# tensorflow/lingvo

Hardware: AMD Instinct MI355X
Metric: train step examples/sec (whole node), Librispeech Conformer-L (higher is better)
Workload: dtype bf16; 1 GPU; model=Conformer-L (17 blocks, d=512, h=8, kernel 32) + LSTM attention decoder, global_batch=512, seq_len=1200, parallelism=dp1, step_mode=hipgraph

## Files before the change

### lingvo_amd/core/py_utils.py

```python

from __future__ import annotations

import contextlib
import math
import threading
from typing import Any, List, Optional, Sequence, Tuple, Union

import torch

from lingvo_amd.core.hyperparams import Params
from lingvo_amd.core.nested_map import NestedMap


class WeightInit:

  @staticmethod
  def _Spec(method: str, scale: float) -> Params:
    p = Params()
    p.Define('method', method, 'Initialization method.')
    p.Define('scale', scale, 'Initialization scale.')
    return p

  @staticmethod
  def Gaussian(scale: float = 1.0) -> Params:
    return WeightInit._Spec('gaussian', scale)

  @staticmethod
  def Uniform(scale: float = 1.0) -> Params:
    return WeightInit._Spec('uniform', scale)

  @staticmethod
  def Constant(scale: float = 0.0) -> Params:
    return WeightInit._Spec('constant', scale)

  @staticmethod
  def Xavier(scale: float = 1.0) -> Params:
    return WeightInit._Spec('xavier', scale)

  @staticmethod
  def GeoMeanXavier(scale: float = 1.0) -> Params:
    return WeightInit._Spec('geo_mean_xavier', scale)

  @staticmethod
  def TruncatedGaussian(scale: float = 1.0) -> Params:
    return WeightInit._Spec('truncated_gaussian', scale)

  @staticmethod
  def GaussianSqrtDim(scale: float = 1.0) -> Params:
    return WeightInit._Spec('gaussian_sqrt_dim', scale)

  @staticmethod
  def UniformSqrtDim(scale: float = 1.0) -> Params:
    return WeightInit._Spec('uniform_sqrt_dim', scale)

  @staticmethod
  def UniformUnitScaling(scale: float = 1.0) -> Params:
    return WeightInit._Spec('uniform_unit_scaling', scale)

  @staticmethod
  def TruncatedGaussianSqrtFanIn(scale: float = 1.0) -> Params:
    return WeightInit._Spec('truncated_gaussian_sqrt_fanin', scale)

  @staticmethod
  def TruncatedGaussianSqrtFanOut(scale: float = 1.0) -> Params:
    return WeightInit._Spec('truncated_gaussian_sqrt_fanout', scale)


def WeightParams(shape: Sequence[int],
                 init: Optional[Params] = None,
                 dtype: torch.dtype = torch.float32,
                 collections: Optional[List[str]] = None) -> Params:
  p = Params()
  p.Define('shape', list(shape), 'Weight shape.')
  p.Define('init', init or WeightInit.Xavier(1.0), 'Initialization spec.')
  p.Define('dtype', dtype, 'Weight dtype.')
  p.Define('collections', collections or [], 'Weight collections.')
  return p


def _FanInFanOut(shape: Sequence[int]) -> Tuple[int, int]:
  if not shape:
    return 1, 1
  if len(shape) == 1:
    return shape[0], shape[0]
  receptive = 1
  for d in shape[:-2]:
    receptive *= d
  return shape[-2] * receptive, shape[-1] * receptive


def InitWeight(shape: Sequence[int], spec: Params,
               generator: Optional[torch.Generator] = None,
               dtype: torch.dtype = torch.float32) -> torch.Tensor:
  method, scale = spec.method, spec.scale
  shape = list(shape)
  dim0 = shape[0] if shape else 1
  fan_in, fan_out = _FanInFanOut(shape)

  def randn():
    return torch.randn(shape, generator=generator, dtype=torch.float32)

  def rand():
    return torch.rand(shape, generator=generator, dtype=torch.float32) * 2 - 1

  if method == 'constant':
    w = torch.full(shape, float(scale), dtype=torch.float32)
  elif method == 'gaussian':
    w = randn() * scale
  elif method == 'uniform':
    w = rand() * scale
  elif method == 'gaussian_sqrt_dim':
    w = randn() * (scale / math.sqrt(max(dim0, 1)))
  elif method == 'uniform_sqrt_dim':
    w = rand() * (scale / math.sqrt(max(dim0, 1)))
  elif method == 'xavier':
    limit = scale * math.sqrt(6.0 / (fan_in + fan_out))
    w = rand() * limit
  elif method == 'geo_mean_xavier':
    limit = scale * math.sqrt(3.0 / math.sqrt(fan_in * fan_out))
    w = rand() * limit
  elif method == 'uniform_unit_scaling':
    w = rand() * (scale * math.sqrt(3.0 / max(fan_in, 1)))
  elif method in ('truncated_gaussian', 'truncated_gaussian_sqrt_fanin',
                  'truncated_gaussian_sqrt_fanout'):
    std = scale
    if method.endswith('fanin'):
      std = scale / math.sqrt(max(fan_in, 1))
    elif method.endswith('fanout'):
      std = scale / math.sqrt(max(fan_out, 1))
    w = torch.empty(shape, dtype=torch.float32)
    torch.nn.init.trunc_normal_(w, std=std, a=-2 * std, b=2 * std,
                                generator=generator)
  else:
    raise ValueError(f'Unknown init method {method!r}')
  return w.to(dtype)


_RNG_STATE = threading.local()


def _GetRngStack() -> List[NestedMap]:
  if not hasattr(_RNG_STATE, 'stack'):
    _RNG_STATE.stack = [NestedMap(global_seed=1234, step=0, op_counter=[0])]
  return _RNG_STATE.stack


@contextlib.contextmanager
def StepSeedScope(global_seed: int, step: int):
  stack = _GetRngStack()
  stack.append(NestedMap(global_seed=int(global_seed), step=int(step),
                         op_counter=[0]))
  if torch.cuda.is_available():
    from lingvo_amd.ops import dropout as dropout_ops
    dropout_ops.SetStepSeed(int(step), int(global_seed))
  try:
    yield
  finally:
    stack.pop()


def GenerateStepSeedPair(op_seed: Optional[int] = None) -> Tuple[int, int]:
  top = _GetRngStack()[-1]
  if op_seed is None:
    op_seed = top.op_counter[0]
    top.op_counter[0] += 1
  mixed = (top.global_seed * 1000003 + op_seed) & 0x7FFFFFFF
  return mixed, top.step


def MakeStepGenerator(device: Union[str, torch.device],
                      op_seed: Optional[int] = None) -> torch.Generator:
  s1, s2 = GenerateStepSeedPair(op_seed)
  g = torch.Generator(device=device)
  g.manual_seed((s1 * 2654435761 + s2) & 0x7FFFFFFFFFFFFFFF)
  return g


def DeterministicDropout(x: torch.Tensor, keep_prob: float,
                         op_seed: Optional[int] = None,
                         act: str = 'NONE') -> torch.Tensor:
  if keep_prob >= 1.0:
    if act == 'SWISH':
      return torch.nn.functional.silu(x)
    if act == 'RELU':
      return torch.relu(x)
    return x
  if x.is_cuda and x.numel() % 8 == 0:
    from lingvo_amd.ops import dropout as dropout_ops
    s1, _ = GenerateStepSeedPair(op_seed)
    return dropout_ops.dropout(x, keep_prob, s1, act=act)
  if act == 'SWISH':
    x = torch.nn.functional.silu(x)
  elif act == 'RELU':
    x = torch.relu(x)
  g = MakeStepGenerator(x.device, op_seed)
  mask = (torch.rand(x.shape, generator=g, device=x.device,
                     dtype=torch.float32) < keep_prob)
  return x * mask.to(x.dtype) / keep_prob


def DeterministicDropoutAdd(x: torch.Tensor, keep_prob: float,
                            residual: torch.Tensor,
                            op_seed: Optional[int] = None,
                            scale: float = 1.0,
                            paddings: Optional[torch.Tensor] = None
                            ) -> torch.Tensor:
  if keep_prob >= 1.0:
    if scale != 1.0:
      x = x * scale
    if paddings is not None:
      x = ApplyPadding(paddings, x)
    return residual + x
  if x.is_cuda and x.numel() % 8 == 0 and \
      (paddings is None or x.shape[-1] % 8 == 0):
    from lingvo_amd.ops import dropout as dropout_ops
    s1, _ = GenerateStepSeedPair(op_seed)
    return dropout_ops.dropout(x, keep_prob, s1, residual=residual,
                               scale=scale, paddings=paddings)
  if scale != 1.0:
    x = x * scale
  if paddings is not None:
    x = ApplyPadding(paddings, x)
  return residual + DeterministicDropout(x, keep_prob, op_seed)


def PaddingsFromLengths(lengths: torch.Tensor, maxlen: int) -> torch.Tensor:
  pos = torch.arange(maxlen, device=lengths.device)[None, :]
  return (pos >= lengths[:, None]).float()


def LengthsFromPaddings(paddings: torch.Tensor) -> torch.Tensor:
  return (1.0 - paddings).sum(dim=1).round().long()


def ApplyPadding(padding: torch.Tensor, x: torch.Tensor,
                 padded_value: float = 0.0) -> torch.Tensor:
  while padding.dim() < x.dim():
    padding = padding.unsqueeze(-1)
  padding = padding.to(x.dtype)
  if padded_value == 0.0:
    return x * (1.0 - padding)
  return x * (1.0 - padding) + padded_value * padding


def PadSequenceDimension(x: torch.Tensor, length: int, pad_val: float = 0.0,
                         axis: int = 1) -> torch.Tensor:
  cur = x.shape[axis]
  if cur == length:
    return x
  if cur > length:
    raise ValueError(f'Cannot pad dim {axis} from {cur} down to {length}')
  pad_shape = list(x.shape)
  pad_shape[axis] = length - cur
  pad = torch.full(pad_shape, pad_val, dtype=x.dtype, device=x.device)
  return torch.cat([x, pad], dim=axis)


def ConcatenatePaddedSequences(x: torch.Tensor, y: torch.Tensor,
                               px: torch.Tensor, py: torch.Tensor
                               ) -> Tuple[torch.Tensor, torch.Tensor]:
  b = x.shape[0]
  lx = LengthsFromPaddings(px)
  ly = LengthsFromPaddings(py)
  tot = int((lx + ly).max().item())
  feat = x.shape[2:]
  out = torch.zeros((b, tot) + tuple(feat), dtype=x.dtype, device=x.device)
  pout = torch.ones((b, tot), dtype=px.dtype, device=px.device)
  for i in range(b):
    n1, n2 = int(lx[i]), int(ly[i])
    out[i, :n1] = x[i, :n1]
    out[i, n1:n1 + n2] = y[i, :n2]
    pout[i, :n1 + n2] = 0.0
  return out, pout


def TrimTrailingPaddings(x: torch.Tensor, paddings: torch.Tensor):
  lengths = LengthsFromPaddings(paddings)
  max_len = int(lengths.max().item()) if lengths.numel() else 0
  max_len = max(max_len, 1)
  return x[:, :max_len], paddings[:, :max_len]


def ReversePaddedSequence(x: torch.Tensor,
                          paddings: torch.Tensor) -> torch.Tensor:
  b, t = paddings.shape
  lengths = LengthsFromPaddings(paddings).to(torch.long)
  pos = torch.arange(t, device=x.device).unsqueeze(0).expand(b, t)
  rev = (lengths.unsqueeze(1) - 1 - pos).clamp_min(0)
  idx = torch.where(pos < lengths.unsqueeze(1), rev, pos)
  shaped = idx.reshape(b, t, *([1] * (x.dim() - 2))).expand_as(x)
  return torch.gather(x, 1, shaped)


def ShiftLeft(x: torch.Tensor, shift: int,
              pad_val: float = 0.0) -> torch.Tensor:
  if shift <= 0:
    return x
  pad = x.new_full((x.shape[0], shift, *x.shape[2:]), pad_val)
  return torch.cat([x[:, shift:], pad], dim=1)


def MixByWeight(fns, weights, seed: Optional[int] = None):
  import random as _random
  rng = _random.Random(seed)
  total = float(sum(weights))
  r = rng.uniform(0.0, total)
  acc = 0.0
  for i, (fn, w) in enumerate(zip(fns, weights)):
    acc += float(w)
    if r <= acc:
      return fn(), i
  return fns[-1](), len(fns) - 1


def SplitRecursively(x, num_splits: int, axis: int = -1):
  if isinstance(x, torch.Tensor):
    assert x.shape[axis] % num_splits == 0
    return list(x.chunk(num_splits, dim=axis))
  if isinstance(x, (list, tuple)):
    split_elems = [SplitRecursively(e, num_splits, axis) for e in x]
    return [type(x)(parts[i] for parts in split_elems)
            for i in range(num_splits)]
  if isinstance(x, NestedMap):
    flat = x.Flatten()
    split_flat = [SplitRecursively(e, num_splits, axis) for e in flat]
    return [x.Pack([parts[i] for parts in split_flat])
            for i in range(num_splits)]
  raise TypeError('Unsupported type for SplitRecursively: %r' % type(x))


def CheckNumerics(x: torch.Tensor, message: str = '') -> torch.Tensor:
  if not torch.isfinite(x).all():
    raise FloatingPointError(f'Tensor has NaN/Inf: {message}')
  return x


def HasNanOrInf(nmap_or_tensor) -> bool:
  if isinstance(nmap_or_tensor, torch.Tensor):
    return not bool(torch.isfinite(nmap_or_tensor).all())
  tensors = [v for v in nmap_or_tensor.Flatten()
             if isinstance(v, torch.Tensor) and v.is_floating_point()]
  return any(not bool(torch.isfinite(t).all()) for t in tensors)


def GlobalGradNorm(grads: List[torch.Tensor]) -> torch.Tensor:
  if not grads:
    return torch.zeros(())
  norms = torch._foreach_norm([g.detach() for g in grads], 2)
  return torch.stack([n.float() for n in norms]).norm(2)


def WeightedAvg(values: torch.Tensor, weights: torch.Tensor
                ) -> Tuple[torch.Tensor, torch.Tensor]:
  w = weights.float()
  total = w.sum()
  avg = (values.float() * w).sum() / total.clamp_min(1e-8)
  return avg, total


def WeightedAvgOfMetrics(metrics_list: List[NestedMap]) -> NestedMap:
  ret = NestedMap()
  if not metrics_list:
    return ret
  for name in metrics_list[0].keys():
    vals = torch.stack([torch.as_tensor(m[name][0]).float()
                        for m in metrics_list])
    wts = torch.stack([torch.as_tensor(m[name][1]).float()
                       for m in metrics_list])
    total_w = wts.sum()
    avg = (vals * wts).sum() / total_w.clamp_min(1e-8)
    ret[name] = (avg, total_w)
  return ret


def ToScalar(x) -> float:
  if isinstance(x, torch.Tensor):
    return float(x.detach().cpu().item())
  return float(x)


def AddVn(theta: NestedMap, vn_std: float) -> NestedMap:

  def add_noise(t):
    if isinstance(t, torch.Tensor) and t.is_floating_point() and \
        t.requires_grad:
      u = GraphSafeUniform(t.shape, t.device).clamp(1e-6, 1 - 1e-6)
      normal = torch.erfinv(2 * u - 1) * math.sqrt(2.0)
      return t + vn_std * normal.to(t.dtype)
    return t

  return theta.Transform(add_noise)


def GraphSafeUniform(shape, device, op_seed: Optional[int] = None
                     ) -> torch.Tensor:
  import math as _math
  n = 1
  for d in shape:
    n *= int(d)
  s1, s2 = GenerateStepSeedPair(op_seed)
  if not (isinstance(device, torch.device) and device.type == 'cuda') and \
      str(device) != 'cuda' and not str(device).startswith('cuda'):
    g = torch.Generator()
    g.manual_seed((s1 * 2654435761 + s2) & 0x7FFFFFFFFFFFFFFF)
    return torch.rand(shape, generator=g)
  from lingvo_amd.ops import dropout as dropout_ops
  buf = dropout_ops._StepSeedBuf(torch.device(device))

  def lshr(x, k):
    return (x >> k) & ((1 << (64 - k)) - 1)

  idx = torch.arange(n, device=device, dtype=torch.int64)
  h = (idx * 0x9E3779B97F4A7C15) ^ (buf + s1)
  h = h ^ lshr(h, 33)
  h = h * -0xAE502812AA7333
  h = h ^ lshr(h, 33)
  h = h * -0x3B314601E57A13AD
  h = h ^ lshr(h, 33)
  u = (h & 0x7FFFFFFF).float() / float(1 << 31)
  return u.reshape(shape)


def MatmulBias(x: torch.Tensor, w: torch.Tensor,
               b: Optional[torch.Tensor] = None) -> torch.Tensor:
  shape = x.shape
  x2 = x.reshape(-1, shape[-1])
  if b is None:
    out = torch.matmul(x2, w)
  else:
    out = torch.addmm(b, x2, w)
  return out.reshape(*shape[:-1], w.shape[-1])


def GlueFusion() -> bool:
  from lingvo_amd.ops import fusion
  return fusion.enabled()


def SetGlueFusion(enabled: bool) -> bool:
  from lingvo_amd.ops import fusion
  return fusion.set_enabled(enabled)


def _CanFuseLinearDropout(x, w, b, keep_prob) -> bool:
  return (GlueFusion() and b is not None and keep_prob < 1.0 and
          x.is_cuda and x.dtype == torch.bfloat16 and
          w.dtype == torch.bfloat16 and b.dtype == torch.bfloat16 and
          w.shape[-1] % 8 == 0 and x.numel() > 0)


def MatmulBiasDropout(x: torch.Tensor, w: torch.Tensor,
                      b: Optional[torch.Tensor], keep_prob: float,
                      op_seed: Optional[int] = None,
                      act: str = 'NONE') -> torch.Tensor:
  if _CanFuseLinearDropout(x, w, b, keep_prob):
    from lingvo_amd.ops import dropout as dropout_ops
    s1, _ = GenerateStepSeedPair(op_seed)
    return dropout_ops.linear_dropout(x, w, b, keep_prob, s1, act=act)
  return DeterministicDropout(MatmulBias(x, w, b), keep_prob, op_seed,
                              act=act)


def MatmulBiasDropoutAdd(x: torch.Tensor, w: torch.Tensor,
                         b: Optional[torch.Tensor], keep_prob: float,
                         residual: torch.Tensor,
                         op_seed: Optional[int] = None, scale: float = 1.0,
                         paddings: Optional[torch.Tensor] = None
                         ) -> torch.Tensor:
  if _CanFuseLinearDropout(x, w, b, keep_prob) and \
      residual.dtype == torch.bfloat16:
    from lingvo_amd.ops import dropout as dropout_ops
    s1, _ = GenerateStepSeedPair(op_seed)
    return dropout_ops.linear_dropout(x, w, b, keep_prob, s1,
                                      residual=residual, scale=scale,
                                      paddings=paddings)
  return DeterministicDropoutAdd(MatmulBias(x, w, b), keep_prob, residual,
                                 op_seed, scale=scale, paddings=paddings)


class Timer:

  def __init__(self):
    self._total = 0.0
    self._start = None

  def Start(self):
    import time
    self._start = time.perf_counter()
    return self

  def Stop(self):
    import time
    if self._start is not None:
      self._total += time.perf_counter() - self._start
      self._start = None
    return self

  def Duration(self) -> float:
    return self._total

  def __enter__(self):
    return self.Start()

  def __exit__(self, *a):
    self.Stop()


def SinkhornAssignment(scores: torch.Tensor, tau: float = 0.1,
                       n_iters: int = 20) -> torch.Tensor:
  log_alpha = scores / tau
  for _ in range(n_iters):
    log_alpha = log_alpha - torch.logsumexp(log_alpha, dim=-1,
                                            keepdim=True)
    log_alpha = log_alpha - torch.logsumexp(log_alpha, dim=-2,
                                            keepdim=True)
  return torch.exp(log_alpha)


def AssertShapeMatch(tensor: torch.Tensor, pattern) -> torch.Tensor:
  shape = tuple(tensor.shape)
  assert len(shape) == len(pattern), (shape, pattern)
  for got, want in zip(shape, pattern):
    assert want == -1 or got == want, (shape, pattern)
  return tensor


def AssertIdShape(*tensors: torch.Tensor) -> None:
  shapes = {tuple(t.shape) for t in tensors}
  assert len(shapes) == 1, shapes


def EstimateFlops(fn, *args) -> int:
  from torch.profiler import profile, ProfilerActivity
  with profile(activities=[ProfilerActivity.CPU],
               with_flops=True) as prof:
    fn(*args)
  return int(sum(e.flops for e in prof.key_averages() if e.flops))


def RandomPermutationSequence(num: int, batch: int,
                              op_seed: Optional[int] = None
                              ) -> torch.Tensor:
  keys = GraphSafeUniform((batch, num), 'cpu', op_seed)
  return keys.argsort(dim=1)


class CachedCall:

  def __init__(self, fn):
    self._fn = fn
    self._has = False
    self._val = None

  def __call__(self):
    if not self._has:
      self._val = self._fn()
      self._has = True
    return self._val
```

### lingvo_amd/layers/conformer.py

```python

from __future__ import annotations

import os
from typing import Optional

import torch
import torch.nn.functional as F

from lingvo_amd.core import py_utils
from lingvo_amd.core.base_layer import BaseLayer
from lingvo_amd.core.nested_map import NestedMap
from lingvo_amd.layers import attention as attention_lib
from lingvo_amd.layers import bn_layers
from lingvo_amd.layers import layers as lingvo_layers
from lingvo_amd.layers import transformer as transformer_lib
from lingvo_amd.ops import conv1d as conv1d_ops


class LConvLayer(BaseLayer):

  @classmethod
  def Params(cls):
    p = super().Params()
    p.Define('input_dim', 0, 'Model dim.')
    p.Define('kernel_size', 32, 'Depthwise conv kernel size.')
    p.Define('is_causal', False, 'Causal depthwise conv.')
    p.Define('conv_norm', 'group', "One of 'batch'|'group'|'layer'.")
    p.Define('num_groups', 32, 'Groups for group norm.')
    p.Define('dropout_prob', 0.0, 'Output dropout.')
    return p

  def __init__(self, params):
    super().__init__(params)
    p = self.p
    d = p.input_dim
    self.CreateChild('ln', lingvo_layers.LayerNorm.Params().Set(
        input_dim=d))
    self.CreateVariable('pw1_w', py_utils.WeightParams(
        [d, 2 * d], p.params_init, p.dtype))
    self.CreateVariable('pw1_b', py_utils.WeightParams(
        [2 * d], py_utils.WeightInit.Constant(0.0), p.dtype))
    self.CreateVariable('dw_w', py_utils.WeightParams(
        [p.kernel_size, d], p.params_init, p.dtype))
    self.CreateVariable('dw_b', py_utils.WeightParams(
        [d], py_utils.WeightInit.Constant(0.0), p.dtype))
    if p.conv_norm == 'batch':
      self.CreateChild('norm', bn_layers.BatchNormLayer.Params().Set(dim=d))
    elif p.conv_norm == 'group':
      self.CreateChild('norm', bn_layers.GroupNormLayer.Params().Set(
          dim=d, num_groups=p.num_groups))
    else:
      self.CreateChild('norm', lingvo_layers.LayerNorm.Params().Set(
          input_dim=d))
    self.CreateVariable('pw2_w', py_utils.WeightParams(
        [d, d], p.params_init, p.dtype))
    self.CreateVariable('pw2_b', py_utils.WeightParams(
        [d], py_utils.WeightInit.Constant(0.0), p.dtype))

  def FProp(self, theta: NestedMap, inputs: torch.Tensor,
            paddings: Optional[torch.Tensor] = None) -> torch.Tensor:
    p = self.p
    x, residual = transformer_lib.PreLn(self.ln, theta.ln, inputs)
    x = py_utils.MatmulBias(x, theta.pw1_w, theta.pw1_b)
    x = F.glu(x, dim=-1)
    if paddings is not None:
      x = py_utils.ApplyPadding(paddings, x)
    x = conv1d_ops.depthwise_conv1d(x, theta.dw_w, theta.dw_b,
                                    causal=p.is_causal)
    if p.conv_norm == 'layer':
      x = self.norm.FProp(theta.norm, x)
      if paddings is not None:
        x = py_utils.ApplyPadding(paddings, x)
      x = F.silu(x)
    elif p.conv_norm == 'group':
      x = self.norm.FProp(theta.norm, x, paddings, act='SILU')
    else:
      x = self.norm.FProp(theta.norm, x, paddings)
      x = F.silu(x)
    if p.dropout_prob and not self.do_eval:
      return py_utils.MatmulBiasDropoutAdd(
          x, theta.pw2_w, theta.pw2_b, 1.0 - p.dropout_prob, residual,
          paddings=paddings)
    x = py_utils.MatmulBias(x, theta.pw2_w, theta.pw2_b)
    if paddings is not None:
      x = py_utils.ApplyPadding(paddings, x)
    return residual + x

  def InitStreamState(self, batch: int, device, dtype) -> NestedMap:
    p = self.p
    return NestedMap(conv=torch.zeros(batch, p.kernel_size - 1,
                                      p.input_dim, device=device,
                                      dtype=dtype))

  def StreamStep(self, theta: NestedMap, inputs: torch.Tensor,
                 paddings: torch.Tensor, state: NestedMap):
    p = self.p
    assert p.is_causal, 'StreamStep requires a causal LConv'
    x = self.ln.FProp(theta.ln, inputs)
    x = py_utils.MatmulBias(x, theta.pw1_w, theta.pw1_b)
    x = F.glu(x, dim=-1)
    x = py_utils.ApplyPadding(paddings, x)
    full = torch.cat([state.conv.to(x.dtype), x], dim=1)
    y = conv1d_ops.depthwise_conv1d(full, theta.dw_w, theta.dw_b,
                                    causal=True)
    x = y[:, state.conv.shape[1]:]
    new_state = NestedMap(conv=full[:, -(p.kernel_size - 1):]
                          if p.kernel_size > 1 else state.conv)
    if p.conv_norm == 'layer':
      x = self.norm.FProp(theta.norm, x)
      x = py_utils.ApplyPadding(paddings, x)
    else:
      x = self.norm.FProp(theta.norm, x, paddings)
    x = F.silu(x)
    x = py_utils.MatmulBias(x, theta.pw2_w, theta.pw2_b)
    x = py_utils.ApplyPadding(paddings, x)
    return inputs + x, new_state


class ConformerLayer(BaseLayer):

  @classmethod
  def Params(cls):
    p = super().Params()
    p.Define('input_dim', 0, 'Model dim.')
    p.Define('atten_num_heads', 8, 'MHSA heads.')
    p.Define('atten_left_context', -1, 'Local attention left window.')
    p.Define('atten_right_context', -1, 'Local attention right window.')
    p.Define('use_relative_atten', True, 'Clipped rel-pos bias in MHSA.')
    p.Define('rel_pos_clip', 127, 'Rel-pos clip distance.')
    p.Define('fflayer_hidden_dim', 0, 'FFN hidden (0 = 4x).')
    p.Define('kernel_size', 32, 'LConv kernel size.')
    p.Define('is_causal', False, 'Causal conv + attention.')
    p.Define('conv_norm', 'group', 'LConv norm type.')
    p.Define('dropout_prob', 0.0, 'Dropout throughout.')
    p.Define('remat', False, 'Gradient-checkpoint this layer '
             '(reference conformer_layer.py:548 p.remat).')
    p.Define('moe_num_experts', 0,
             'If > 0, the ENDING half-FFN becomes a top-2 MoE FFN '
             '(reference conformer_layer.py:1006 MoE-FFN option).')
    p.Define('moe_capacity_factor', 2.0, 'MoE capacity factor.')
    return p

  @classmethod
  def CommonParams(cls, input_dim, atten_num_heads=8, kernel_size=32,
                   is_causal=False, dropout_prob=0.0):
    return cls.Params().Set(
        input_dim=input_dim, atten_num_heads=atten_num_heads,
        kernel_size=kernel_size, is_causal=is_causal,
        dropout_prob=dropout_prob)

  def __init__(self, params):
    super().__init__(params)
    p = self.p
    d = p.input_dim
    hidden = p.fflayer_hidden_dim or 4 * d
    ff = transformer_lib.TransformerFeedForwardLayer.Params().Set(
        input_dim=d, hidden_dim=hidden, activation='SWISH',
        residual_weight=0.5, residual_dropout_prob=p.dropout_prob,
        relu_dropout_prob=p.dropout_prob)
    self.CreateChild('fflayer_start', ff.Copy())
    if p.moe_num_experts:
      self.CreateChild(
          'fflayer_end',
          transformer_lib.MoETransformerFeedForwardLayer.Params().Set(
              input_dim=d, hidden_dim=hidden,
              num_experts=p.moe_num_experts,
              expert_capacity_factor=p.moe_capacity_factor,
              residual_dropout_prob=p.dropout_prob))
    else:
      self.CreateChild('fflayer_end', ff.Copy())
    atten = transformer_lib.TransformerAttentionLayer.Params().Set(
        input_dim=d, num_heads=p.atten_num_heads, is_masked=p.is_causal,
        residual_dropout_prob=p.dropout_prob)
    atten.atten_tpl.rel_pos_bias = p.use_relative_atten
    atten.atten_tpl.rel_pos_clip = p.rel_pos_clip
    atten.atten_tpl.left_context = p.atten_left_context
    atten.atten_tpl.right_context = p.atten_right_context
    atten.atten_tpl.atten_dropout_prob = p.dropout_prob
    self.CreateChild('trans_atten', atten)
    self.CreateChild('lconv', LConvLayer.Params().Set(
        input_dim=d, kernel_size=p.kernel_size, is_causal=p.is_causal,
        conv_norm=p.conv_norm, dropout_prob=p.dropout_prob))
    self.CreateChild('final_ln', lingvo_layers.LayerNorm.Params().Set(
        input_dim=d))

  def _Body(self, theta, x, paddings):
    x = self.fflayer_start.FProp(theta.fflayer_start, x, paddings)
    x = self.trans_atten.FProp(theta.trans_atten, x, paddings)
    x = self.lconv.FProp(theta.lconv, x, paddings)
    x = self.fflayer_end.FProp(theta.fflayer_end, x, paddings)
    return self.final_ln.FProp(theta.final_ln, x)

  def FProp(self, theta: NestedMap, inputs: torch.Tensor,
            paddings: Optional[torch.Tensor] = None) -> torch.Tensor:
    if self.p.remat and self.training:
      return torch.utils.checkpoint.checkpoint(
          lambda x: self._Body(theta, x, paddings), inputs,
          use_reentrant=False)
    return self._Body(theta, inputs, paddings)

  def InitStreamState(self, theta: NestedMap, batch: int, max_len: int,
                      device, dtype=torch.float32) -> NestedMap:
    assert self.p.is_causal, 'streaming requires a causal block'
    return NestedMap(
        atten=self.trans_atten.InitStates(theta.trans_atten, batch,
                                          max_len, device, dtype),
        lconv=self.lconv.InitStreamState(batch, device, dtype))

  def StreamStep(self, theta: NestedMap, x_chunk: torch.Tensor,
                 paddings_chunk: torch.Tensor, state: NestedMap):
    x = self.fflayer_start.FProp(theta.fflayer_start, x_chunk,
                                 paddings_chunk)
    x, state.atten = self.trans_atten.StreamStep(
        theta.trans_atten, x, paddings_chunk, state.atten)
    x, state.lconv = self.lconv.StreamStep(theta.lconv, x,
                                           paddings_chunk, state.lconv)
    x = self.fflayer_end.FProp(theta.fflayer_end, x, paddings_chunk)
    return self.final_ln.FProp(theta.final_ln, x), state


class _Conv3x3S2Nhwc(torch.autograd.Function):

  CELLS = [
      ((-1, -1), [(0, 0, 1)]),
      ((0, -1), [(1, 0, 0), (2, 0, 1)]),
      ((-1, 0), [(0, 2, 1), (0, 1, 2)]),
      ((0, 0), [(1, 2, 0), (2, 2, 1), (2, 1, 2), (1, 1, 3)]),
  ]

  BLOCKS = [(0, 1), (1, 1), (1, 0), (0, 0)]

  @staticmethod
  def _s2d(x):
    B, H, W, C = x.shape
    Ho, Wo = H // 2, W // 2
    if x.is_cuda and x.dtype == torch.bfloat16 and C % 8 == 0:
      from lingvo_amd.ops import _loader
      X = _loader.get_ext(required=True).s2d_fwd(x)
      return X.reshape(B * (Ho + 1) * (Wo + 1), 4 * C), Ho, Wo
    X = x.new_zeros(B, Ho + 1, Wo + 1, 4 * C)
    for i, (a, b) in enumerate(_Conv3x3S2Nhwc.BLOCKS):
      X[:, 1:, 1:, i * C:(i + 1) * C] = x[:, a::2, b::2, :]
    return X.reshape(B * (Ho + 1) * (Wo + 1), 4 * C), Ho, Wo

  @staticmethod
  def _cell_weight(w, taps, transpose=False):
    mats = [w[dt, df] for (dt, df, _) in
            sorted(taps, key=lambda t: t[2])]
    cat = torch.cat(mats, dim=0)
    return cat.t().contiguous() if transpose else cat.contiguous()

  @staticmethod
  def forward(ctx, x, w, bias):
    B, H, W, C = x.shape
    Co = w.shape[3]
    pad_h, pad_w = H % 2, W % 2
    if pad_h or pad_w:
      x = F.pad(x, (0, 0, 0, pad_w, 0, pad_h))
    Hp2, Wp2 = x.shape[1], x.shape[2]
    X, Ho, Wo = _Conv3x3S2Nhwc._s2d(x)
    Wp = Wo + 1
    Rp = B * (Ho + 1) * Wp
    base = Wp + 1
    O = bias.to(x.dtype).expand(Rp, Co).contiguous()
    for (dtau, dphi), taps in _Conv3x3S2Nhwc.CELLS:
      off = dtau * Wp + dphi
      blks = sorted(t[2] for t in taps)
      k0, k1 = blks[0] * C, (blks[-1] + 1) * C
      wc = _Conv3x3S2Nhwc._cell_weight(w.to(x.dtype), taps)
      O[base:].addmm_(X[base + off:Rp + off, k0:k1], wc)
    ctx.save_for_backward(X, w)
    ctx.dims = (B, H, W, C, Ho, Wo, Co, pad_h, pad_w)
    ctx.bias_dtype = bias.dtype
    out = O.reshape(B, Ho + 1, Wp, Co)[:, 1:, 1:, :]
    return out.contiguous()

  @staticmethod
  def backward(ctx, dout):
    X, w = ctx.saved_tensors
    B, H, W, C, Ho, Wo, Co, pad_h, pad_w = ctx.dims
    Wp = Wo + 1
    Rp = B * (Ho + 1) * Wp
    base = Wp + 1
    dout4 = dout.reshape(B, Ho, Wo, Co)
    if dout.is_cuda and dout.dtype == torch.bfloat16 and Co % 8 == 0:
      from lingvo_amd.ops import _loader
      dO = _loader.get_ext(required=True).pad_scatter(
          dout4.contiguous())
    else:
      dO = dout.new_zeros(B, Ho + 1, Wp, Co)
      dO[:, 1:, 1:, :] = dout4
    dO = dO.reshape(Rp, Co)
    dX = torch.zeros_like(X)
    dw = torch.empty_like(w)
    for (dtau, dphi), taps in _Conv3x3S2Nhwc.CELLS:
      off = dtau * Wp + dphi
      blks = sorted(t[2] for t in taps)
      k0, k1 = blks[0] * C, (blks[-1] + 1) * C
      g = X[base + off:Rp + off, k0:k1].t() @ dO[base:]
      for i, (dt, df, _) in enumerate(sorted(taps,
                                             key=lambda t: t[2])):
        dw[dt, df] = g[i * C:(i + 1) * C].to(w.dtype)
      wc_t = _Conv3x3S2Nhwc._cell_weight(w.to(dO.dtype), taps,
                                         transpose=True)
      dX[base + off:Rp + off, k0:k1].addmm_(dO[base:], wc_t)
    if dX.is_cuda and dX.dtype == torch.bfloat16 and C % 8 == 0:
      from lingvo_amd.ops import _loader
      dx = _loader.get_ext(required=True).s2d_inv(
          dX.reshape(B, Ho + 1, Wp, 4 * C), C)
    else:
      dXr = dX.reshape(B, Ho + 1, Wp, 4 * C)[:, 1:, 1:, :]
      dx_full = dout.new_empty(B, 2 * Ho, 2 * Wo, C)
      for i, (a, b) in enumerate(_Conv3x3S2Nhwc.BLOCKS):
        dx_full[:, a::2, b::2, :] = dXr[..., i * C:(i + 1) * C]
      dx = dx_full
    if pad_h or pad_w:
      dx = dx[:, :2 * Ho - pad_h, :2 * Wo - pad_w, :].contiguous()
    dbias = dO[base:].float().sum(0).to(ctx.bias_dtype)
    return dx, dw, dbias


class ConvSubsampling(BaseLayer):

  @classmethod
  def Params(cls):
    p = super().Params()
    p.Define('input_freq_dim', 80, 'Mel bins.')
    p.Define('channels', 0, 'Conv channels (defaults to output_dim).')
    p.Define('output_dim', 512, 'Output model dim.')
    return p

  def __init__(self, params):
    super().__init__(params)
    p = self.p
    ch = p.channels or p.output_dim
    self._ch = ch
    self.CreateVariable('conv1_w', py_utils.WeightParams(
        [3, 3, 1, ch], p.params_init, p.dtype))
    self.CreateVariable('conv1_b', py_utils.WeightParams(
        [ch], py_utils.WeightInit.Constant(0.0), p.dtype))
    self.CreateVariable('conv2_w', py_utils.WeightParams(
        [3, 3, ch, ch], p.params_init, p.dtype))
    self.CreateVariable('conv2_b', py_utils.WeightParams(
        [ch], py_utils.WeightInit.Constant(0.0), p.dtype))
    freq_out = ((p.input_freq_dim + 1) // 2 + 1) // 2
    self.CreateVariable('proj_w', py_utils.WeightParams(
        [freq_out * ch, p.output_dim], p.params_init, p.dtype))
    self.CreateVariable('proj_b', py_utils.WeightParams(
        [p.output_dim], py_utils.WeightInit.Constant(0.0), p.dtype))

  def FProp(self, theta: NestedMap, inputs: torch.Tensor,
            paddings: torch.Tensor):
    b, t, f = inputs.shape
    ch = self._ch
    cols = F.unfold(inputs.unsqueeze(1), kernel_size=3, stride=2,
                    padding=1)
    h1 = (f + 1) // 2
    t1 = (t + 1) // 2
    x = torch.matmul(cols.transpose(1, 2),
                     theta.conv1_w.reshape(9, ch)) + theta.conv1_b
    x = F.relu(x).reshape(b, t1, h1, ch)
    x = F.relu(_Conv3x3S2Nhwc.apply(x, theta.conv2_w, theta.conv2_b))
    _, t4, f4, _ = x.shape
    x = x.reshape(b, t4, f4 * ch)
    out = torch.addmm(theta.proj_b, x.reshape(-1, f4 * ch),
                      theta.proj_w).reshape(b, t4, -1)
    out_paddings = paddings[:, ::2][:, ::2]
    out_paddings = out_paddings[:, :t4]
    out = py_utils.ApplyPadding(out_paddings, out)
    return out, out_paddings
```

### lingvo_amd/ops/conv1d.py

```python

from __future__ import annotations

from typing import Optional

import torch
import torch.nn.functional as F

from lingvo_amd.ops import _loader


class _DwConv1dFn(torch.autograd.Function):

  @staticmethod
  def forward(ctx, x, w, bias, pad):
    ext = _loader.get_ext(required=True)
    y = ext.dwconv1d_fwd(x, w, bias, pad)
    ctx.save_for_backward(x, w)
    ctx.pad = pad
    ctx.has_bias = bias is not None
    ctx.wdtype = w.dtype
    return y

  @staticmethod
  def backward(ctx, dy):
    ext = _loader.get_ext(required=True)
    x, w = ctx.saved_tensors
    dx, dw, db = ext.dwconv1d_bwd(dy.contiguous(), x, w, ctx.pad)
    return (dx, dw.to(ctx.wdtype),
            db.to(ctx.wdtype) if ctx.has_bias else None, None)


def depthwise_conv1d(x: torch.Tensor, w: torch.Tensor,
                     bias: Optional[torch.Tensor] = None,
                     causal: bool = False) -> torch.Tensor:
  k = w.shape[0]
  pad = k - 1 if causal else (k - 1) // 2
  if x.is_cuda:
    orig = x.dtype
    out = _DwConv1dFn.apply(
        x.to(torch.bfloat16).contiguous(), w.to(torch.bfloat16).contiguous(),
        None if bias is None else bias.to(torch.bfloat16).contiguous(), pad)
    return out.to(orig) if orig != torch.bfloat16 else out
  xf = x.float().permute(0, 2, 1)
  wf = w.float().t().unsqueeze(1)
  left = pad
  right = (k - 1) - pad
  xf = F.pad(xf, (left, right))
  out = F.conv1d(xf, wf, bias.float() if bias is not None else None,
                 groups=x.shape[2])
  return out.permute(0, 2, 1).to(x.dtype)
```

### lingvo_amd/ops/hip/bindings.cpp

```cpp
#include <torch/extension.h>

#include <vector>

std::vector<torch::Tensor> layer_norm_fwd(torch::Tensor x,
                                          torch::Tensor scale,
                                          torch::Tensor bias, double eps,
                                          bool rms);
std::vector<torch::Tensor> layer_norm_bwd(torch::Tensor dy, torch::Tensor x,
                                          torch::Tensor scale,
                                          torch::Tensor mean,
                                          torch::Tensor rstd, bool rms,
                                          c10::optional<torch::Tensor> dres);

torch::Tensor mfma_probe(torch::Tensor a, torch::Tensor bT);
torch::Tensor tr16_probe(torch::Tensor a, torch::Tensor b);

std::vector<torch::Tensor> fa_fwd(torch::Tensor q, torch::Tensor k,
                                  torch::Tensor v,
                                  c10::optional<torch::Tensor> klen,
                                  c10::optional<torch::Tensor> bias,
                                  c10::optional<torch::Tensor> qseg,
                                  c10::optional<torch::Tensor> kseg,
                                  int64_t win_l, int64_t win_r,
                                  int64_t bias_clip, double scale,
                                  int64_t chunk_size, int64_t left_chunks);
std::vector<torch::Tensor> fa_bwd(torch::Tensor dout, torch::Tensor q,
                                  torch::Tensor k, torch::Tensor v,
                                  torch::Tensor o, torch::Tensor lse,
                                  c10::optional<torch::Tensor> klen,
                                  c10::optional<torch::Tensor> bias,
                                  c10::optional<torch::Tensor> qseg,
                                  c10::optional<torch::Tensor> kseg,
                                  bool bias_grad, int64_t win_l,
                                  int64_t win_r, int64_t bias_clip,
                                  double scale, int64_t chunk_size,
                                  int64_t left_chunks,
                                  c10::optional<torch::Tensor> dq_out,
                                  c10::optional<torch::Tensor> dk_out,
                                  c10::optional<torch::Tensor> dv_out,
                                  const std::string& route);

torch::Tensor dwconv1d_fwd(torch::Tensor x, torch::Tensor w,
                           c10::optional<torch::Tensor> bias, int64_t pad);
std::vector<torch::Tensor> dwconv1d_bwd(torch::Tensor dy, torch::Tensor x,
                                        torch::Tensor w, int64_t pad);

std::vector<torch::Tensor> xent_fwd(torch::Tensor logits,
                                    torch::Tensor labels);
torch::Tensor xent_bwd(torch::Tensor logits, torch::Tensor labels,
                       torch::Tensor lse, torch::Tensor gout);

torch::Tensor dropout_fwd(torch::Tensor x, c10::optional<torch::Tensor> res,
                          int64_t seed,
                          c10::optional<torch::Tensor> step_seed,
                          double keep, int64_t act, double scale,
                          c10::optional<torch::Tensor> pad, int64_t d);
torch::Tensor dropout_bwd(torch::Tensor dy, c10::optional<torch::Tensor> x,
                          int64_t seed,
                          c10::optional<torch::Tensor> step_seed,
                          double keep, int64_t act, double scale,
                          c10::optional<torch::Tensor> pad, int64_t d);
std::vector<torch::Tensor> dropout_bwd_colsum(
    torch::Tensor dy, c10::optional<torch::Tensor> x, int64_t seed,
    c10::optional<torch::Tensor> step_seed, double keep, int64_t act,
    double scale, c10::optional<torch::Tensor> pad, int64_t d);

std::vector<torch::Tensor> group_norm_fwd(torch::Tensor x,
                                          torch::Tensor gamma,
                                          torch::Tensor beta,
                                          c10::optional<torch::Tensor> pad,
                                          int64_t groups, double eps,
                                          int64_t act);
std::vector<torch::Tensor> group_norm_bwd(torch::Tensor dy, torch::Tensor x,
                                          torch::Tensor gamma,
                                          torch::Tensor beta,
                                          c10::optional<torch::Tensor> pad,
                                          torch::Tensor mean,
                                          torch::Tensor rstd,
                                          int64_t groups, int64_t act);

std::vector<torch::Tensor> lstm_gates_fwd_op(torch::Tensor gates,
                                             torch::Tensor c0, double fgb,
                                             double cap);
std::vector<torch::Tensor> lstm_gates_bwd_op(
    torch::Tensor gates, torch::Tensor c0, torch::Tensor c1,
    torch::Tensor dm1, c10::optional<torch::Tensor> dc1, double fgb,
    double cap);

void RegisterInputPipeline(py::module_& m);

void RegisterWpmTokenizer(py::module_& m);

void RegisterRecordBatcher(py::module_& m);

torch::Tensor emb_gather(torch::Tensor table, torch::Tensor ids,
                         double scale);
torch::Tensor emb_scatter_add(torch::Tensor dy, torch::Tensor ids,
                              int64_t vocab, double scale);

std::vector<torch::Tensor> moe_positions(torch::Tensor top1,
                                         torch::Tensor top2,
                                         int64_t num_experts);

torch::Tensor s2d_fwd(torch::Tensor x);
torch::Tensor s2d_inv(torch::Tensor dX, int64_t C);
torch::Tensor pad_scatter(torch::Tensor dout);

std::vector<torch::Tensor> topk_rows(torch::Tensor scores, int64_t k);

void smallm_gemm(torch::Tensor a, torch::Tensor wt,
                 c10::optional<torch::Tensor> pre, torch::Tensor out,
                 int64_t k, int64_t wt_col0, double alpha,
                 int64_t pre_mode);
std::vector<torch::Tensor> attend_fwd(torch::Tensor q, torch::Tensor enc,
                                      torch::Tensor pad, double scale);
std::vector<torch::Tensor> attend_bwd(torch::Tensor dctx,
                                      torch::Tensor probs, torch::Tensor q,
                                      torch::Tensor enc, torch::Tensor denc,
                                      double scale);
int64_t attend_lds_limit();
int64_t attend_lds_bytes(int64_t s, int64_t d, bool bwd);

void lstm_scan_fwd(torch::Tensor gates, torch::Tensor c, torch::Tensor m,
                   torch::Tensor pad, torch::Tensor wmt, int64_t rev_mask,
                   double fgb, double cap, int64_t s_begin, int64_t s_end,
                   int64_t rows_per_block);
void lstm_scan_bwd(torch::Tensor gates, torch::Tensor c, torch::Tensor pad,
                   torch::Tensor wm, c10::optional<torch::Tensor> dm_out,
                   c10::optional<torch::Tensor> dc_out,
                   torch::Tensor dgates, torch::Tensor dc_carry,
                   torch::Tensor dm_pass, int64_t rev_mask, double fgb,
                   double cap, int64_t s_begin, int64_t s_end,
                   int64_t rows_per_block);

std::vector<torch::Tensor> ctc_fwd(torch::Tensor logits,
                                   torch::Tensor logit_lengths,
                                   torch::Tensor labels,
                                   torch::Tensor label_lengths,
                                   int64_t blank);
torch::Tensor ctc_bwd(torch::Tensor logits, torch::Tensor logit_lengths,
                      torch::Tensor labels, torch::Tensor label_lengths,
                      torch::Tensor lse, torch::Tensor emis,
                      torch::Tensor alpha, torch::Tensor beta,
                      torch::Tensor nll, torch::Tensor valid,
                      torch::Tensor gout, int64_t blank);
int64_t ctc_max_label_len();

std::vector<torch::Tensor> rnnt_fwd(torch::Tensor logits,
                                    torch::Tensor logit_lengths,
                                    torch::Tensor labels,
                                    torch::Tensor label_lengths,
                                    int64_t blank);
torch::Tensor rnnt_bwd(torch::Tensor logits, torch::Tensor logit_lengths,
                       torch::Tensor labels, torch::Tensor label_lengths,
                       torch::Tensor lse, torch::Tensor emis,
                       torch::Tensor alpha, torch::Tensor beta,
                       torch::Tensor valid, torch::Tensor gnll,
                       int64_t blank);
int64_t rnnt_max_label_len();

PYBIND11_MODULE(TORCH_EXTENSION_NAME, m) {
  RegisterInputPipeline(m);
  RegisterWpmTokenizer(m);
  RegisterRecordBatcher(m);
  m.def("group_norm_fwd", &group_norm_fwd, "Fused padded GroupNorm fwd");
  m.def("group_norm_bwd", &group_norm_bwd, "Fused padded GroupNorm bwd");
  m.def("lstm_gates_fwd", &lstm_gates_fwd_op, "Fused LSTM gates fwd");
  m.def("lstm_gates_bwd", &lstm_gates_bwd_op, "Fused LSTM gates bwd");
  m.def("dropout_fwd", &dropout_fwd, "Fused dropout fwd");
  m.def("dropout_bwd", &dropout_bwd, "Fused dropout bwd");
  m.def("dropout_bwd_colsum", &dropout_bwd_colsum,
        "Fused dropout bwd + fp32 column sums of dx");
  m.def("xent_fwd", &xent_fwd, "Fused softmax-xent fwd");
  m.def("xent_bwd", &xent_bwd, "Fused softmax-xent bwd");
  m.def("dwconv1d_fwd", &dwconv1d_fwd, "Depthwise time conv fwd");
  m.def("dwconv1d_bwd", &dwconv1d_bwd, "Depthwise time conv bwd");
  m.def("layer_norm_fwd", &layer_norm_fwd, "Fused LayerNorm/RMSNorm fwd");
  m.def("layer_norm_bwd", &layer_norm_bwd, "Fused LayerNorm/RMSNorm bwd",
        py::arg("dy"), py::arg("x"), py::arg("scale"), py::arg("mean"),
        py::arg("rstd"), py::arg("rms"), py::arg("dres") = py::none());
  m.def("mfma_probe", &mfma_probe, "MFMA 16x16x32 layout probe");
  m.def("tr16_probe", &tr16_probe, "ds_read_tr16_b64 layout probe");
  m.def("fa_fwd", &fa_fwd, "Flash attention forward");
  m.def("fa_bwd", &fa_bwd, "Flash attention backward", py::arg("dout"),
        py::arg("q"), py::arg("k"), py::arg("v"), py::arg("o"),
        py::arg("lse"), py::arg("klen"), py::arg("bias"), py::arg("qseg"),
        py::arg("kseg"), py::arg("bias_grad"), py::arg("win_l"),
        py::arg("win_r"), py::arg("bias_clip"), py::arg("scale"),
        py::arg("chunk_size"), py::arg("left_chunks"),
        py::arg("dq_out") = py::none(), py::arg("dk_out") = py::none(),
        py::arg("dv_out") = py::none(), py::arg("route") = "auto");
  m.def("emb_gather", &emb_gather, "Embedding gather fwd");
  m.def("emb_scatter_add", &emb_scatter_add,
        "Deterministic embedding scatter-add bwd");
  m.def("moe_positions", &moe_positions,
        "Deterministic MoE top-2 position scan");
  m.def("smallm_gemm", &smallm_gemm,
        "Small-M MFMA GEMM (decode-step projections)");
  m.def("attend_fwd", &attend_fwd, "Fused dot-attention step fwd");
  m.def("attend_bwd", &attend_bwd, "Fused dot-attention step bwd");
  m.def("attend_lds_limit", &attend_lds_limit,
        "Dynamic LDS bytes an attend_* launch may ask for on this device");
  m.def("attend_lds_bytes", &attend_lds_bytes,
        "Dynamic LDS bytes attend_fwd/attend_bwd ask for at (S, D)");
  m.def("lstm_scan_fwd", &lstm_scan_fwd,
        "Fused LSTM scan forward: one launch per step, all directions");
  m.def("lstm_scan_bwd", &lstm_scan_bwd,
        "Fused LSTM scan backward: one launch per step, all directions");
  m.def("ctc_fwd", &ctc_fwd,
        "CTC loss forward: nll, valid and the backward's workspaces");
  m.def("ctc_bwd", &ctc_bwd, "CTC loss backward: dlogits");
  m.def("ctc_max_label_len", &ctc_max_label_len,
        "Largest label width L the CTC kernels support");
  m.def("rnnt_fwd", &rnnt_fwd,
        "Transducer loss forward: nll, valid and the backward's workspaces");
  m.def("rnnt_bwd", &rnnt_bwd, "Transducer loss backward: dlogits");
  m.def("rnnt_max_label_len", &rnnt_max_label_len,
        "Largest label width U the transducer kernels support");
  m.def("s2d_fwd", &s2d_fwd, "Space-to-depth + pad (conv frontend)");
  m.def("topk_rows", &topk_rows, "Row-wise top-k (beam pruning, K12)");
  m.def("s2d_inv", &s2d_inv, "Inverse space-to-depth");
  m.def("pad_scatter", &pad_scatter, "Zero-border pad scatter");
}
```

### lingvo_amd/ops/hip/common.h

```cpp
#pragma once

#include <hip/hip_runtime.h>
#include <hip/hip_bf16.h>
#include <hip/hip_fp16.h>

#define WAVE_SIZE 64

#define LV_CHECK_HIP(expr)                                       \
  do {                                                           \
    hipError_t _e = (expr);                                      \
    if (_e != hipSuccess) {                                      \
      TORCH_CHECK(false, "HIP error: ", hipGetErrorString(_e));  \
    }                                                            \
  } while (0)

typedef __attribute__((ext_vector_type(4))) float floatx4;
typedef __attribute__((ext_vector_type(8))) float floatx8;
typedef __attribute__((ext_vector_type(8))) unsigned short ushortx8;
typedef __attribute__((ext_vector_type(4))) unsigned short ushortx4;
typedef __attribute__((ext_vector_type(2))) unsigned short ushortx2;

__device__ __forceinline__ float bf16_bits_to_float(unsigned short u) {
  union {
    unsigned int i;
    float f;
  } v;
  v.i = ((unsigned int)u) << 16;
  return v.f;
}

__device__ __forceinline__ unsigned short float_to_bf16_bits(float f) {
  __hip_bfloat16 h = __float2bfloat16(f);
  union {
    __hip_bfloat16 h;
    unsigned short u;
  } v;
  v.h = h;
  return v.u;
}

__device__ __forceinline__ float wave_reduce_sum(float x) {
#pragma unroll
  for (int off = 32; off > 0; off >>= 1) {
    x += __shfl_xor(x, off, WAVE_SIZE);
  }
  return x;
}

__device__ __forceinline__ float wave_reduce_max(float x) {
#pragma unroll
  for (int off = 32; off > 0; off >>= 1) {
    x = fmaxf(x, __shfl_xor(x, off, WAVE_SIZE));
  }
  return x;
}

template <int NWAVES>
__device__ __forceinline__ float block_reduce_sum(float x, float* scratch) {
  const int lane = threadIdx.x & (WAVE_SIZE - 1);
  const int wid = threadIdx.x / WAVE_SIZE;
  x = wave_reduce_sum(x);
  if (lane == 0) scratch[wid] = x;
  __syncthreads();
  float total = 0.f;
#pragma unroll
  for (int i = 0; i < NWAVES; ++i) total += scratch[i];
  __syncthreads();
  return total;
}

__device__ __forceinline__ int cdiv_dev(int a, int b) { return (a + b - 1) / b; }

static inline int cdiv(long a, long b) { return (int)((a + b - 1) / b); }

static inline int memory_bound_grid(long total_work, int block_size,
                                    int cap_blocks = 2048) {
  long want = (total_work + block_size - 1) / block_size;
  return (int)(want < cap_blocks ? (want > 0 ? want : 1) : cap_blocks);
}
```

### lingvo_amd/ops/hip/conv1d.hip

```cpp

#include <ATen/cuda/CUDAContext.h>
#include <torch/extension.h>

#include "common.h"

namespace {

constexpr int MAXK = 33;

template <int KT>
__global__ void dwconv_fwd(const unsigned short* __restrict__ x,
                           const unsigned short* __restrict__ w,
                           const unsigned short* __restrict__ bias,
                           unsigned short* __restrict__ y, int B, int T,
                           int D, int Krt, int pad) {
  const int K = KT > 0 ? KT : Krt;
  const long nvec = (long)B * T * (D / 8);
  const int dvec = D / 8;
  for (long i = (long)blockIdx.x * blockDim.x + threadIdx.x; i < nvec;
       i += (long)gridDim.x * blockDim.x) {
    const int dv = (int)(i % dvec);
    const long bt = i / dvec;
    const int t = (int)(bt % T);
    const long b = bt / T;
    float acc[8];
    if (bias) {
      ushortx8 bv = *reinterpret_cast<const ushortx8*>(bias + dv * 8);
#pragma unroll
      for (int e = 0; e < 8; ++e) acc[e] = bf16_bits_to_float(bv[e]);
    } else {
#pragma unroll
      for (int e = 0; e < 8; ++e) acc[e] = 0.f;
    }
#pragma unroll
    for (int j = 0; j < (KT > 0 ? KT : 1); ++j) {
      if (KT == 0) break;
      int ts = t + j - pad;
      if (ts < 0 || ts >= T) continue;
      ushortx8 xv = *reinterpret_cast<const ushortx8*>(
          x + (b * T + ts) * D + dv * 8);
      ushortx8 wv = *reinterpret_cast<const ushortx8*>(w + j * D + dv * 8);
#pragma unroll
      for (int e = 0; e < 8; ++e)
        acc[e] += bf16_bits_to_float(xv[e]) * bf16_bits_to_float(wv[e]);
    }
    if (KT == 0) {
      for (int j = 0; j < K; ++j) {
        int ts = t + j - pad;
        if (ts < 0 || ts >= T) continue;
        ushortx8 xv = *reinterpret_cast<const ushortx8*>(
            x + (b * T + ts) * D + dv * 8);
        ushortx8 wv =
            *reinterpret_cast<const ushortx8*>(w + j * D + dv * 8);
#pragma unroll
        for (int e = 0; e < 8; ++e)
          acc[e] += bf16_bits_to_float(xv[e]) * bf16_bits_to_float(wv[e]);
      }
    }
    ushortx8 ov;
#pragma unroll
    for (int e = 0; e < 8; ++e) ov[e] = float_to_bf16_bits(acc[e]);
    *reinterpret_cast<ushortx8*>(y + (b * T + t) * D + dv * 8) = ov;
  }
}

template <int KT, int R>
__global__ __launch_bounds__(256) void dwconv_fwd_reg(
    const unsigned short* __restrict__ x,
    const unsigned short* __restrict__ w,
    const unsigned short* __restrict__ bias,
    unsigned short* __restrict__ y, int B, int T, int D, int pad) {
  const int dvec = D / 8;
  const int tblks = (T + R - 1) / R;
  const long nwork = (long)B * tblks * dvec;
  for (long i = (long)blockIdx.x * blockDim.x + threadIdx.x; i < nwork;
       i += (long)gridDim.x * blockDim.x) {
    const int dv = (int)(i % dvec);
    const long bt = i / dvec;
    const int t0 = (int)(bt % tblks) * R;
    const long b = bt / tblks;
    ushortx8 wv[KT];
#pragma unroll
    for (int j = 0; j < KT; ++j) {
      wv[j] = *reinterpret_cast<const ushortx8*>(w + j * D + dv * 8);
    }
    float acc[R][8];
#pragma unroll
    for (int r = 0; r < R; ++r) {
      if (bias) {
        ushortx8 bv = *reinterpret_cast<const ushortx8*>(bias + dv * 8);
#pragma unroll
        for (int e = 0; e < 8; ++e) acc[r][e] = bf16_bits_to_float(bv[e]);
      } else {
#pragma unroll
        for (int e = 0; e < 8; ++e) acc[r][e] = 0.f;
      }
    }
    const long rowbase = b * T;
    auto loadx = [&](int t) -> ushortx8 {
      ushortx8 v;
      if (t >= 0 && t < T) {
        v = *reinterpret_cast<const ushortx8*>(
            x + (rowbase + t) * D + dv * 8);
      } else {
#pragma unroll
        for (int e = 0; e < 8; ++e) v[e] = 0;
      }
      return v;
    };
    ushortx8 W[R];
#pragma unroll
    for (int r = 0; r < R; ++r) W[r] = loadx(t0 + r - pad);
#pragma unroll
    for (int j = 0; j < KT; ++j) {
#pragma unroll
      for (int r = 0; r < R; ++r) {
#pragma unroll
        for (int e = 0; e < 8; ++e) {
          acc[r][e] += bf16_bits_to_float(W[r][e]) *
                       bf16_bits_to_float(wv[j][e]);
        }
      }
      if (j + 1 < KT) {
#pragma unroll
        for (int r = 0; r + 1 < R; ++r) W[r] = W[r + 1];
        W[R - 1] = loadx(t0 + (R - 1) + (j + 1) - pad);
      }
    }
#pragma unroll
    for (int r = 0; r < R; ++r) {
      const int t = t0 + r;
      if (t >= T) continue;
      ushortx8 ov;
#pragma unroll
      for (int e = 0; e < 8; ++e) ov[e] = float_to_bf16_bits(acc[r][e]);
      *reinterpret_cast<ushortx8*>(y + (rowbase + t) * D + dv * 8) = ov;
    }
  }
}

template <int KT>
__global__ void dwconv_bwd_dx(const unsigned short* __restrict__ dy,
                              const unsigned short* __restrict__ w,
                              unsigned short* __restrict__ dx, int B, int T,
                              int D, int Krt, int pad) {
  const int K = KT > 0 ? KT : Krt;
  const long nvec = (long)B * T * (D / 8);
  const int dvec = D / 8;
  for (long i = (long)blockIdx.x * blockDim.x + threadIdx.x; i < nvec;
       i += (long)gridDim.x * blockDim.x) {
    const int dv = (int)(i % dvec);
    const long bt = i / dvec;
    const int t = (int)(bt % T);
    const long b = bt / T;
    float acc[8];
#pragma unroll
    for (int e = 0; e < 8; ++e) acc[e] = 0.f;
#pragma unroll
    for (int j = 0; j < (KT > 0 ? KT : 1); ++j) {
      if (KT == 0) break;
      int ty = t - j + pad;
      if (ty < 0 || ty >= T) continue;
      ushortx8 gv = *reinterpret_cast<const ushortx8*>(
          dy + (b * T + ty) * D + dv * 8);
      ushortx8 wv = *reinterpret_cast<const ushortx8*>(w + j * D + dv * 8);
#pragma unroll
      for (int e = 0; e < 8; ++e)
        acc[e] += bf16_bits_to_float(gv[e]) * bf16_bits_to_float(wv[e]);
    }
    if (KT == 0) {
      for (int j = 0; j < K; ++j) {
        int ty = t - j + pad;
        if (ty < 0 || ty >= T) continue;
        ushortx8 gv = *reinterpret_cast<const ushortx8*>(
            dy + (b * T + ty) * D + dv * 8);
        ushortx8 wv =
            *reinterpret_cast<const ushortx8*>(w + j * D + dv * 8);
#pragma unroll
        for (int e = 0; e < 8; ++e)
          acc[e] += bf16_bits_to_float(gv[e]) * bf16_bits_to_float(wv[e]);
      }
    }
    ushortx8 ov;
#pragma unroll
    for (int e = 0; e < 8; ++e) ov[e] = float_to_bf16_bits(acc[e]);
    *reinterpret_cast<ushortx8*>(dx + (b * T + t) * D + dv * 8) = ov;
  }
}

constexpr int DW_CHUNK = 64;
constexpr int DW_DBLK = 128;

__global__ __launch_bounds__(256) void dwconv_bwd_dw(
    const unsigned short* __restrict__ dy,
    const unsigned short* __restrict__ x,
    float* __restrict__ dw_part,
    float* __restrict__ db_part,
    int B, int T, int D, int K, int pad,
    int ngroups) {
  __shared__ unsigned short x_s[DW_CHUNK + MAXK - 1][DW_DBLK + 8];
  __shared__ unsigned short dy_s[DW_CHUNK][DW_DBLK + 8];
  const int tid = threadIdx.x;
  const int dg = tid & 15;
  const int tq = (tid >> 4) & 3;
  const int rq = tid >> 6;
  const int d0 = blockIdx.x * DW_DBLK + dg * 8;
  const long rows = (long)B * T;
  const int xrows = DW_CHUNK + K - 1;

  float dw8[8][8];
#pragma unroll
  for (int jj = 0; jj < 8; ++jj) {
#pragma unroll
    for (int e = 0; e < 8; ++e) dw8[jj][e] = 0.f;
  }
  float db8[8] = {0, 0, 0, 0, 0, 0, 0, 0};

  const long nchunks = (rows + DW_CHUNK - 1) / DW_CHUNK;
  for (long c = blockIdx.y; c < nchunks; c += ngroups) {
    const long r0 = c * DW_CHUNK;
    for (int i = tid; i < xrows * (DW_DBLK / 8); i += 256) {
      int row = i / (DW_DBLK / 8);
      int d8 = (i % (DW_DBLK / 8)) * 8;
      long fr = r0 - pad + row;
      ushortx8 v;
      int gd = blockIdx.x * DW_DBLK + d8;
      if (fr >= 0 && fr < rows && gd + 7 < D) {
        v = *reinterpret_cast<const ushortx8*>(x + fr * D + gd);
      } else {
        for (int e = 0; e < 8; ++e) v[e] = 0;
      }
      *reinterpret_cast<ushortx8*>(&x_s[row][d8]) = v;
    }
    for (int i = tid; i < DW_CHUNK * (DW_DBLK / 8); i += 256) {
      int row = i / (DW_DBLK / 8);
      int d8 = (i % (DW_DBLK / 8)) * 8;
      long fr = r0 + row;
      ushortx8 v;
      int gd = blockIdx.x * DW_DBLK + d8;
      if (fr < rows && gd + 7 < D) {
        v = *reinterpret_cast<const ushortx8*>(dy + fr * D + gd);
      } else {
        for (int e = 0; e < 8; ++e) v[e] = 0;
      }
      *reinterpret_cast<ushortx8*>(&dy_s[row][d8]) = v;
    }
    __syncthreads();

    const int nrows = (int)min((long)DW_CHUNK, rows - r0);
    const int lr_hi = min((rq + 1) * 16, nrows);
    for (int lr = rq * 16; lr < lr_hi; ++lr) {
      ushortx8 gv = *reinterpret_cast<const ushortx8*>(&dy_s[lr][dg * 8]);
      float g[8];
#pragma unroll
      for (int e = 0; e < 8; ++e) g[e] = bf16_bits_to_float(gv[e]);
      const int t = (int)((r0 + lr) % T);
      if (tq == 0) {
#pragma unroll
        for (int e = 0; e < 8; ++e) db8[e] += g[e];
      }
#pragma unroll
      for (int jj = 0; jj < 8; ++jj) {
        const int j = tq * 8 + jj;
        if (j >= K) break;
        const int ts = t + j - pad;
        if (ts < 0 || ts >= T) continue;
        ushortx8 xv =
            *reinterpret_cast<const ushortx8*>(&x_s[lr + j][dg * 8]);
#pragma unroll
        for (int e = 0; e < 8; ++e) {
          dw8[jj][e] += g[e] * bf16_bits_to_float(xv[e]);
        }
      }
    }
    __syncthreads();
  }

  __shared__ float dw_lds[MAXK - 1][DW_DBLK];
  __shared__ float db_lds[DW_DBLK];
  for (int i = tid; i < K * DW_DBLK; i += 256) {
    dw_lds[i / DW_DBLK][i % DW_DBLK] = 0.f;
  }
  for (int i = tid; i < DW_DBLK; i += 256) db_lds[i] = 0.f;
  __syncthreads();
#pragma unroll
  for (int jj = 0; jj < 8; ++jj) {
    const int j = tq * 8 + jj;
    if (j >= K) break;
#pragma unroll
    for (int e = 0; e < 8; ++e) {
      if (dw8[jj][e] != 0.f) atomicAdd(&dw_lds[j][dg * 8 + e], dw8[jj][e]);
    }
  }
  if (tq == 0) {
#pragma unroll
    for (int e = 0; e < 8; ++e) {
      if (db8[e] != 0.f) atomicAdd(&db_lds[dg * 8 + e], db8[e]);
    }
  }
  __syncthreads();
  const long gbase = (long)blockIdx.y * K * D;
  for (int i = tid; i < K * DW_DBLK; i += 256) {
    const int j = i / DW_DBLK;
    const int d = blockIdx.x * DW_DBLK + i % DW_DBLK;
    if (d < D) dw_part[gbase + (long)j * D + d] = dw_lds[j][i % DW_DBLK];
  }
  for (int i = tid; i < DW_DBLK; i += 256) {
    const int d = blockIdx.x * DW_DBLK + i;
    if (d < D) db_part[(long)blockIdx.y * D + d] = db_lds[i];
  }
}

__global__ void dwconv_bwd_dw_reduce(const float* __restrict__ dw_part,
                                     const float* __restrict__ db_part,
                                     float* __restrict__ dw,
                                     float* __restrict__ db, long kd, int D,
                                     int ngroups) {
  for (long i = (long)blockIdx.x * blockDim.x + threadIdx.x; i < kd + D;
       i += (long)gridDim.x * blockDim.x) {
    float sum = 0.f;
    if (i < kd) {
      for (int g = 0; g < ngroups; ++g) sum += dw_part[(long)g * kd + i];
      dw[i] = sum;
    } else {
      const long d = i - kd;
      for (int g = 0; g < ngroups; ++g) sum += db_part[(long)g * D + d];
      db[d] = sum;
    }
  }
}

}

torch::Tensor dwconv1d_fwd(torch::Tensor x, torch::Tensor w,
                           c10::optional<torch::Tensor> bias, int64_t pad) {
  TORCH_CHECK(x.is_cuda() && x.is_contiguous() && x.dim() == 3 &&
              x.scalar_type() == torch::kBFloat16, "x must be bf16 [B,T,D]");
  TORCH_CHECK(x.size(2) % 8 == 0, "D must be divisible by 8");
  const int B = x.size(0), T = x.size(1), D = x.size(2), K = w.size(0);
  TORCH_CHECK(K < MAXK, "kernel size < ", MAXK);
  auto y = torch::empty_like(x);
  auto stream = at::cuda::getCurrentCUDAStream();
  long nvec = (long)B * T * (D / 8);
  int grid = memory_bound_grid(nvec, 256);
  static const bool use_reg = []() {
    const char* e = getenv("LINGVO_DWCONV_REG");
    return e && e[0] == '1';
  }();
  if (use_reg && K == 32) {
    long nwork = (long)B * ((T + 3) / 4) * (D / 8);
    hipLaunchKernelGGL((dwconv_fwd_reg<32, 4>),
                       dim3(memory_bound_grid(nwork, 256)), dim3(256), 0,
                       stream, (const unsigned short*)x.data_ptr(),
                       (const unsigned short*)w.data_ptr(),
                       bias.has_value() ? (const unsigned short*)
                                              bias->data_ptr()
                                        : nullptr,
                       (unsigned short*)y.data_ptr(), B, T, D, (int)pad);
    return y;
  }
  auto fwd_kern = dwconv_fwd<0>;
  hipLaunchKernelGGL(fwd_kern, dim3(grid), dim3(256), 0, stream,
                     (const unsigned short*)x.data_ptr(),
                     (const unsigned short*)w.data_ptr(),
                     bias.has_value() ? (const unsigned short*)
                                            bias->data_ptr()
                                      : nullptr,
                     (unsigned short*)y.data_ptr(), B, T, D, K, (int)pad);
  return y;
}

std::vector<torch::Tensor> dwconv1d_bwd(torch::Tensor dy, torch::Tensor x,
                                        torch::Tensor w, int64_t pad) {
  const int B = x.size(0), T = x.size(1), D = x.size(2), K = w.size(0);
  auto dx = torch::empty_like(x);
  auto opts = x.options().dtype(torch::kFloat32);
  auto dw = torch::zeros({K, D}, opts);
  auto db = torch::zeros({D}, opts);
  auto stream = at::cuda::getCurrentCUDAStream();
  long nvec = (long)B * T * (D / 8);
  auto dx_kern = dwconv_bwd_dx<0>;
  hipLaunchKernelGGL(dx_kern, dim3(memory_bound_grid(nvec, 256)),
                     dim3(256), 0, stream,
                     (const unsigned short*)dy.data_ptr(),
                     (const unsigned short*)w.data_ptr(),
                     (unsigned short*)dx.data_ptr(), B, T, D, K, (int)pad);
  long nchunks = ((long)B * T + DW_CHUNK - 1) / DW_CHUNK;
  int dblks = (D + DW_DBLK - 1) / DW_DBLK;
  int ngroups = (int)std::min<long>(std::max<long>(1, 1024 / dblks),
                                    nchunks);
  auto dw_part = torch::empty({(long)ngroups * K * D}, opts);
  auto db_part = torch::empty({(long)ngroups * D}, opts);
  dim3 grid_w(dblks, ngroups);
  hipLaunchKernelGGL(dwconv_bwd_dw, grid_w, dim3(256), 0, stream,
                     (const unsigned short*)dy.data_ptr(),
                     (const unsigned short*)x.data_ptr(),
                     dw_part.data_ptr<float>(), db_part.data_ptr<float>(),
                     B, T, D, K, (int)pad, ngroups);
  const long kd = (long)K * D;
  hipLaunchKernelGGL(dwconv_bwd_dw_reduce,
                     dim3((int)std::min<long>((kd + D + 255) / 256, 1024)),
                     dim3(256), 0, stream, dw_part.data_ptr<float>(),
                     db_part.data_ptr<float>(), dw.data_ptr<float>(),
                     db.data_ptr<float>(), kd, D, ngroups);
  return {dx, dw, db};
}
```

### lingvo_amd/ops/hip/dropout.hip

```cpp

#include <ATen/cuda/CUDAContext.h>
#include <torch/extension.h>

#include "common.h"

namespace {

__device__ __forceinline__ unsigned int hash_u32(unsigned long long seed,
                                                 unsigned long long idx) {
  unsigned long long h = seed ^ (idx * 0x9E3779B97F4A7C15ull);
  h ^= h >> 33;
  h *= 0xFF51AFD7ED558CCDull;
  h ^= h >> 33;
  h *= 0xC4CEB9FE1A85EC53ull;
  h ^= h >> 33;
  return (unsigned int)h;
}

template <int ACT>
__device__ __forceinline__ float apply_act(float v) {
  if (ACT == 1) return v / (1.f + __expf(-v)) ;
  if (ACT == 2) return v > 0.f ? v : 0.f;
  return v;
}

template <int ACT>
__device__ __forceinline__ float act_grad(float v) {
  if (ACT == 1) {
    const float s = 1.f / (1.f + __expf(-v));
    return s * (1.f + v * (1.f - s));
  }
  if (ACT == 2) return v > 0.f ? 1.f : 0.f;
  return 1.f;
}

template <bool RESIDUAL, int ACT>
__global__ void dropout_fwd_kernel(const unsigned short* __restrict__ x,
                                   const unsigned short* __restrict__ res,
                                   unsigned short* __restrict__ y,
                                   long nvec, unsigned long long seed,
                                   const long* __restrict__ step_seed,
                                   float keep, float inv_keep,
                                   float scale,
                                   const unsigned short* __restrict__ pad,
                                   long dvec) {
  const unsigned int thresh = (unsigned int)(keep * 4294967296.0);
  if (step_seed) seed ^= (unsigned long long)(*step_seed);
  for (long i = (long)blockIdx.x * blockDim.x + threadIdx.x; i < nvec;
       i += (long)gridDim.x * blockDim.x) {
    float sc = scale;
    if (pad) sc *= 1.f - bf16_bits_to_float(pad[i / dvec]);
    ushortx8 v = *reinterpret_cast<const ushortx8*>(x + i * 8);
    ushortx8 o;
#pragma unroll
    for (int e = 0; e < 8; ++e) {
      bool kept = hash_u32(seed, i * 8 + e) < thresh;
      float f = kept ? apply_act<ACT>(bf16_bits_to_float(v[e])) * inv_keep
                           * sc
                     : 0.f;
      o[e] = float_to_bf16_bits(f);
    }
    if (RESIDUAL) {
      ushortx8 r = *reinterpret_cast<const ushortx8*>(res + i * 8);
#pragma unroll
      for (int e = 0; e < 8; ++e)
        o[e] = float_to_bf16_bits(bf16_bits_to_float(o[e]) +
                                  bf16_bits_to_float(r[e]));
    }
    *reinterpret_cast<ushortx8*>(y + i * 8) = o;
  }
}

template <int ACT>
__device__ __forceinline__ ushortx8 dropout_bwd_vec(
    const unsigned short* __restrict__ dy, const unsigned short* __restrict__ x,
    long i, unsigned long long seed, unsigned int thresh, float inv_keep,
    float sc) {
  ushortx8 v = *reinterpret_cast<const ushortx8*>(dy + i * 8);
  ushortx8 xv;
  if (ACT != 0) xv = *reinterpret_cast<const ushortx8*>(x + i * 8);
  ushortx8 o;
#pragma unroll
  for (int e = 0; e < 8; ++e) {
    bool kept = hash_u32(seed, i * 8 + e) < thresh;
    float f = kept ? bf16_bits_to_float(v[e]) * inv_keep * sc : 0.f;
    if (ACT != 0) f *= act_grad<ACT>(bf16_bits_to_float(xv[e]));
    o[e] = float_to_bf16_bits(f);
  }
  return o;
}

template <int ACT>
__global__ void dropout_bwd_kernel(const unsigned short* __restrict__ dy,
                                   const unsigned short* __restrict__ x,
                                   unsigned short* __restrict__ dx,
                                   long nvec, unsigned long long seed,
                                   const long* __restrict__ step_seed,
                                   float keep, float inv_keep,
                                   float scale,
                                   const unsigned short* __restrict__ pad,
                                   long dvec) {
  const unsigned int thresh = (unsigned int)(keep * 4294967296.0);
  if (step_seed) seed ^= (unsigned long long)(*step_seed);
  for (long i = (long)blockIdx.x * blockDim.x + threadIdx.x; i < nvec;
       i += (long)gridDim.x * blockDim.x) {
    float sc = scale;
    if (pad) sc *= 1.f - bf16_bits_to_float(pad[i / dvec]);
    *reinterpret_cast<ushortx8*>(dx + i * 8) =
        dropout_bwd_vec<ACT>(dy, x, i, seed, thresh, inv_keep, sc);
  }
}

constexpr int kColsumWaves = 4;
constexpr int kColsumCols = WAVE_SIZE * 8;

template <int ACT>
__global__ __launch_bounds__(WAVE_SIZE * kColsumWaves)
void dropout_bwd_colsum_kernel(const unsigned short* __restrict__ dy,
                               const unsigned short* __restrict__ x,
                               unsigned short* __restrict__ dx,
                               float* __restrict__ partials, long rows,
                               long dvec, long rows_per_block,
                               unsigned long long seed,
                               const long* __restrict__ step_seed, float keep,
                               float inv_keep, float scale,
                               const unsigned short* __restrict__ pad) {
  __shared__ float red[kColsumWaves][kColsumCols];
  const unsigned int thresh = (unsigned int)(keep * 4294967296.0);
  if (step_seed) seed ^= (unsigned long long)(*step_seed);
  const int lane = threadIdx.x & (WAVE_SIZE - 1);
  const int wave = threadIdx.x / WAVE_SIZE;
  const long cv = (long)blockIdx.x * WAVE_SIZE + lane;
  const long r0 = (long)blockIdx.y * rows_per_block;
  const long r1 = min(rows, r0 + rows_per_block);
  float acc[8];
#pragma unroll
  for (int e = 0; e < 8; ++e) acc[e] = 0.f;
  if (cv < dvec) {
    for (long r = r0 + wave; r < r1; r += kColsumWaves) {
      const long i = r * dvec + cv;
      float sc = scale;
      if (pad) sc *= 1.f - bf16_bits_to_float(pad[r]);
      ushortx8 o = dropout_bwd_vec<ACT>(dy, x, i, seed, thresh, inv_keep, sc);
      *reinterpret_cast<ushortx8*>(dx + i * 8) = o;
#pragma unroll
      for (int e = 0; e < 8; ++e) acc[e] += bf16_bits_to_float(o[e]);
    }
  }
#pragma unroll
  for (int e = 0; e < 8; ++e) red[wave][lane * 8 + e] = acc[e];
  __syncthreads();
  const long D = dvec * 8;
  for (int c = threadIdx.x; c < kColsumCols; c += blockDim.x) {
    const long col = (long)blockIdx.x * kColsumCols + c;
    if (col < D) {
      float s = 0.f;
#pragma unroll
      for (int w = 0; w < kColsumWaves; ++w) s += red[w][c];
      partials[(long)blockIdx.y * D + col] = s;
    }
  }
}

__global__ __launch_bounds__(256)
void colsum_reduce_kernel(const float* __restrict__ partials,
                          float* __restrict__ out, int nslab, long D) {
  __shared__ float red[64][16];
  const int q = threadIdx.x & 3;
  const int slice = threadIdx.x >> 2;
  const long col = (long)blockIdx.x * 16 + q * 4;
  floatx4 s = {0.f, 0.f, 0.f, 0.f};
  if (col < D) {
    for (int p = slice; p < nslab; p += 64)
      s += *reinterpret_cast<const floatx4*>(partials + (long)p * D + col);
  }
#pragma unroll
  for (int j = 0; j < 4; ++j) red[slice][q * 4 + j] = s[j];
  __syncthreads();
  if (threadIdx.x < 16) {
    const long c = (long)blockIdx.x * 16 + threadIdx.x;
    if (c < D) {
      float t = 0.f;
      for (int p = 0; p < 64; ++p) t += red[p][threadIdx.x];
      out[c] = t;
    }
  }
}

}

torch::Tensor dropout_fwd(torch::Tensor x, c10::optional<torch::Tensor> res,
                          int64_t seed, c10::optional<torch::Tensor> step_seed,
                          double keep, int64_t act, double scale,
                          c10::optional<torch::Tensor> pad, int64_t d) {
  TORCH_CHECK(x.is_cuda() && x.is_contiguous() &&
              x.scalar_type() == torch::kBFloat16 && x.numel() % 8 == 0);
  TORCH_CHECK(!(res.has_value() && act != 0),
              "residual+activation fusion unsupported");
  TORCH_CHECK(!pad.has_value() || (d > 0 && d % 8 == 0),
              "padding fusion needs D % 8 == 0");
  auto y = torch::empty_like(x);
  long nvec = x.numel() / 8;
  auto stream = at::cuda::getCurrentCUDAStream();
  const long* ssp = step_seed.has_value() ?
      step_seed->data_ptr<long>() : nullptr;
  const unsigned short* pp = pad.has_value() ?
      (const unsigned short*)pad->data_ptr() : nullptr;
  const long dvec = d > 0 ? d / 8 : 1;
#define LAUNCH_FWD(RES, ACT, RESPTR)                                         \
  hipLaunchKernelGGL((dropout_fwd_kernel<RES, ACT>),                         \
                     dim3(memory_bound_grid(nvec, 256)), dim3(256), 0,       \
                     stream, (const unsigned short*)x.data_ptr(), RESPTR,    \
                     (unsigned short*)y.data_ptr(), nvec,                    \
                     (unsigned long long)seed, ssp, (float)keep,             \
                     (float)(1.0 / keep), (float)scale, pp, dvec)
  if (res.has_value()) {
    LAUNCH_FWD(true, 0, (const unsigned short*)res->data_ptr());
  } else if (act == 1) {
    LAUNCH_FWD(false, 1, nullptr);
  } else if (act == 2) {
    LAUNCH_FWD(false, 2, nullptr);
  } else {
    LAUNCH_FWD(false, 0, nullptr);
  }
#undef LAUNCH_FWD
  return y;
}

torch::Tensor dropout_bwd(torch::Tensor dy, c10::optional<torch::Tensor> x,
                          int64_t seed, c10::optional<torch::Tensor> step_seed,
                          double keep, int64_t act, double scale,
                          c10::optional<torch::Tensor> pad, int64_t d) {
  TORCH_CHECK(act == 0 || x.has_value(),
              "activation-fused dropout bwd needs the pre-activation input");
  auto dx = torch::empty_like(dy);
  long nvec = dy.numel() / 8;
  auto stream = at::cuda::getCurrentCUDAStream();
  const long* ssp = step_seed.has_value() ?
      step_seed->data_ptr<long>() : nullptr;
  const unsigned short* xp = x.has_value() ?
      (const unsigned short*)x->data_ptr() : nullptr;
  const unsigned short* pp = pad.has_value() ?
      (const unsigned short*)pad->data_ptr() : nullptr;
  const long dvec = d > 0 ? d / 8 : 1;
#define LAUNCH_BWD(ACT)                                                      \
  hipLaunchKernelGGL((dropout_bwd_kernel<ACT>),                              \
                     dim3(memory_bound_grid(nvec, 256)), dim3(256), 0,       \
                     stream, (const unsigned short*)dy.data_ptr(), xp,       \
                     (unsigned short*)dx.data_ptr(), nvec,                   \
                     (unsigned long long)seed, ssp, (float)keep,             \
                     (float)(1.0 / keep), (float)scale, pp, dvec)
  if (act == 1) {
    LAUNCH_BWD(1);
  } else if (act == 2) {
    LAUNCH_BWD(2);
  } else {
    LAUNCH_BWD(0);
  }
#undef LAUNCH_BWD
  return dx;
}

std::vector<torch::Tensor> dropout_bwd_colsum(
    torch::Tensor dy, c10::optional<torch::Tensor> x, int64_t seed,
    c10::optional<torch::Tensor> step_seed, double keep, int64_t act,
    double scale, c10::optional<torch::Tensor> pad, int64_t d) {
  TORCH_CHECK(dy.is_cuda() && dy.is_contiguous() &&
              dy.scalar_type() == torch::kBFloat16,
              "dy must be contiguous CUDA bf16");
  TORCH_CHECK(d > 0 && d % 8 == 0 && dy.numel() % d == 0,
              "column sums need D % 8 == 0 and numel % D == 0");
  TORCH_CHECK(act == 0 || x.has_value(),
              "activation-fused dropout bwd needs the pre-activation input");
  const long rows = dy.numel() / d;
  TORCH_CHECK(!x.has_value() ||
              (x->is_cuda() && x->is_contiguous() &&
               x->scalar_type() == torch::kBFloat16 &&
               x->numel() == dy.numel()), "x must match dy");
  TORCH_CHECK(!pad.has_value() ||
              (pad->is_cuda() && pad->is_contiguous() &&
               pad->scalar_type() == torch::kBFloat16 &&
               pad->numel() == rows), "pad must be [rows] bf16");
  auto dx = torch::empty_like(dy);
  auto fopts = dy.options().dtype(torch::kFloat32);
  auto colsum = torch::empty({d}, fopts);
  if (rows == 0) {
    colsum.zero_();
    return {dx, colsum};
  }
  const long dvec = d / 8;
  const int gx = cdiv(dvec, WAVE_SIZE);
  const long want_y = std::max<long>(1, 2048 / gx);
  long rpb = (rows + want_y - 1) / want_y;
  rpb = (rpb + kColsumWaves - 1) / kColsumWaves * kColsumWaves;
  const int gy = cdiv(rows, rpb);
  auto partials = torch::empty({(long)gy, (long)d}, fopts);
  auto stream = at::cuda::getCurrentCUDAStream();
  const long* ssp = step_seed.has_value() ?
      step_seed->data_ptr<long>() : nullptr;
  const unsigned short* xp = x.has_value() ?
      (const unsigned short*)x->data_ptr() : nullptr;
  const unsigned short* pp = pad.has_value() ?
      (const unsigned short*)pad->data_ptr() : nullptr;
#define LAUNCH_BWD_CS(ACT)                                                   \
  hipLaunchKernelGGL((dropout_bwd_colsum_kernel<ACT>), dim3(gx, gy),         \
                     dim3(WAVE_SIZE * kColsumWaves), 0, stream,              \
                     (const unsigned short*)dy.data_ptr(), xp,               \
                     (unsigned short*)dx.data_ptr(),                         \
                     partials.data_ptr<float>(), rows, dvec, rpb,            \
                     (unsigned long long)seed, ssp, (float)keep,             \
                     (float)(1.0 / keep), (float)scale, pp)
  if (act == 1) {
    LAUNCH_BWD_CS(1);
  } else if (act == 2) {
    LAUNCH_BWD_CS(2);
  } else {
    LAUNCH_BWD_CS(0);
  }
#undef LAUNCH_BWD_CS
  hipLaunchKernelGGL(colsum_reduce_kernel, dim3(cdiv(d, 16)), dim3(256), 0,
                     stream, partials.data_ptr<float>(),
                     colsum.data_ptr<float>(), gy, (long)d);
  return {dx, colsum};
}
```

### lingvo_amd/ops/hip/group_norm.hip

```cpp

#include <ATen/cuda/CUDAContext.h>
#include <torch/extension.h>

#include "common.h"

namespace {

constexpr int GN_BLOCK = 256;
constexpr int GN_WAVES = GN_BLOCK / WAVE_SIZE;

__global__ __launch_bounds__(GN_BLOCK) void gn_fwd_kernel(
    const unsigned short* __restrict__ x,
    const unsigned short* __restrict__ gamma,
    const unsigned short* __restrict__ beta,
    const unsigned short* __restrict__ paddings,
    unsigned short* __restrict__ y, float* __restrict__ mean_out,
    float* __restrict__ rstd_out, int B, int T, int D, int G, float eps,
    int act) {
  __shared__ float scratch[GN_WAVES];
  const int b = blockIdx.x / G;
  const int g = blockIdx.x % G;
  const int cg = D / G;
  const int tid = threadIdx.x;

  float sum = 0.f, sumsq = 0.f, count = 0.f;
  for (int i = tid; i < T * cg; i += GN_BLOCK) {
    int t = i / cg;
    int c = g * cg + i % cg;
    float pad = paddings ? bf16_bits_to_float(paddings[(long)b * T + t])
                         : 0.f;
    if (pad < 0.5f) {
      float v = bf16_bits_to_float(x[((long)b * T + t) * D + c]);
      sum += v;
      sumsq += v * v;
      count += 1.f;
    }
  }
  sum = block_reduce_sum<GN_WAVES>(sum, scratch);
  sumsq = block_reduce_sum<GN_WAVES>(sumsq, scratch);
  count = block_reduce_sum<GN_WAVES>(count, scratch);
  count = fmaxf(count, 1.f);
  float mu = sum / count;
  float var = sumsq / count - mu * mu;
  float rstd = rsqrtf(var + eps);
  if (tid == 0) {
    mean_out[(long)b * G + g] = mu;
    rstd_out[(long)b * G + g] = rstd;
  }

  for (int i = tid; i < T * cg; i += GN_BLOCK) {
    int t = i / cg;
    int c = g * cg + i % cg;
    float pad = paddings ? bf16_bits_to_float(paddings[(long)b * T + t])
                         : 0.f;
    float v = bf16_bits_to_float(x[((long)b * T + t) * D + c]);
    float w = 1.f + bf16_bits_to_float(gamma[c]);
    float bb = bf16_bits_to_float(beta[c]);
    float out = (v - mu) * rstd * w + bb;
    if (act == 1) out = out / (1.f + __expf(-out));
    out *= (1.f - pad);
    y[((long)b * T + t) * D + c] = float_to_bf16_bits(out);
  }
}

__global__ __launch_bounds__(GN_BLOCK) void gn_bwd_kernel(
    const unsigned short* __restrict__ dy,
    const unsigned short* __restrict__ x,
    const unsigned short* __restrict__ gamma,
    const unsigned short* __restrict__ beta,
    const unsigned short* __restrict__ paddings,
    const float* __restrict__ mean, const float* __restrict__ rstd,
    unsigned short* __restrict__ dx, float* __restrict__ dgamma,
    float* __restrict__ dbeta, int B, int T, int D, int G, int act) {
  __shared__ float scratch[GN_WAVES];
  const int b = blockIdx.x / G;
  const int g = blockIdx.x % G;
  const int cg = D / G;
  const int tid = threadIdx.x;
  const float mu = mean[(long)b * G + g];
  const float rs = rstd[(long)b * G + g];

  __shared__ float dg_s[64];
  __shared__ float db_s[64];
  for (int i = tid; i < cg; i += GN_BLOCK) {
    dg_s[i] = 0.f;
    db_s[i] = 0.f;
  }
  __syncthreads();
  float s1 = 0.f, s2 = 0.f, count = 0.f;
  for (int i = tid; i < T * cg; i += GN_BLOCK) {
    int t = i / cg;
    int ci = i % cg;
    int c = g * cg + ci;
    float pad = paddings ? bf16_bits_to_float(paddings[(long)b * T + t])
                         : 0.f;
    if (pad < 0.5f) {
      float xv = bf16_bits_to_float(x[((long)b * T + t) * D + c]);
      float dyv = bf16_bits_to_float(dy[((long)b * T + t) * D + c]);
      float w = 1.f + bf16_bits_to_float(gamma[c]);
      float xhat = (xv - mu) * rs;
      float dxhat = dyv * w;
      s1 += dxhat;
      s2 += dxhat * xhat;
      count += 1.f;
      atomicAdd(&dg_s[ci], dyv * xhat);
      atomicAdd(&db_s[ci], dyv);
    }
  }
  s1 = block_reduce_sum<GN_WAVES>(s1, scratch);
  s2 = block_reduce_sum<GN_WAVES>(s2, scratch);
  count = block_reduce_sum<GN_WAVES>(count, scratch);
  count = fmaxf(count, 1.f);
  const float inv_n = 1.f / count;

  for (int i = tid; i < cg; i += GN_BLOCK) {
    int c = g * cg + i;
    if (dg_s[i] != 0.f) atomicAdd(dgamma + c, dg_s[i]);
    if (db_s[i] != 0.f) atomicAdd(dbeta + c, db_s[i]);
  }

  for (int i = tid; i < T * cg; i += GN_BLOCK) {
    int t = i / cg;
    int c = g * cg + i % cg;
    float pad = paddings ? bf16_bits_to_float(paddings[(long)b * T + t])
                         : 0.f;
    float xv = bf16_bits_to_float(x[((long)b * T + t) * D + c]);
    float dyv = bf16_bits_to_float(dy[((long)b * T + t) * D + c]);
    float w = 1.f + bf16_bits_to_float(gamma[c]);
    float xhat = (xv - mu) * rs;
    float dxhat = dyv * w;
    float val = rs * (dxhat - inv_n * (s1 + xhat * s2)) * (1.f - pad);
    dx[((long)b * T + t) * D + c] = float_to_bf16_bits(val);
  }
}

__global__ __launch_bounds__(GN_BLOCK) void gn_bwd_vec_kernel(
    const unsigned short* __restrict__ dy,
    const unsigned short* __restrict__ x,
    const unsigned short* __restrict__ gamma,
    const unsigned short* __restrict__ beta,
    const unsigned short* __restrict__ paddings,
    const float* __restrict__ mean, const float* __restrict__ rstd,
    unsigned short* __restrict__ dx, float* __restrict__ dgamma,
    float* __restrict__ dbeta, int B, int T, int D, int G, int act) {
  __shared__ float scratch[GN_WAVES];
  __shared__ float dg_s[64];
  __shared__ float db_s[64];
  const int b = blockIdx.x / G;
  const int g = blockIdx.x % G;
  const int cg = D / G;
  const int noct = cg / 8;
  const int tid = threadIdx.x;
  const int oct = tid % noct;
  const int rt = tid / noct;
  const int rstep = GN_BLOCK / noct;
  const float mu = mean[(long)b * G + g];
  const float rs = rstd[(long)b * G + g];
  const long col0 = (long)g * cg + oct * 8;

  float w[8], bb[8];
  {
    ushortx8 gv = *reinterpret_cast<const ushortx8*>(gamma + col0);
    ushortx8 bv = *reinterpret_cast<const ushortx8*>(beta + col0);
#pragma unroll
    for (int e = 0; e < 8; ++e) {
      w[e] = 1.f + bf16_bits_to_float(gv[e]);
      bb[e] = bf16_bits_to_float(bv[e]);
    }
  }
  for (int i = tid; i < cg; i += GN_BLOCK) {
    dg_s[i] = 0.f;
    db_s[i] = 0.f;
  }

  float s1 = 0.f, s2 = 0.f, count = 0.f;
  float dg8[8], db8[8];
#pragma unroll
  for (int e = 0; e < 8; ++e) {
    dg8[e] = 0.f;
    db8[e] = 0.f;
  }
  for (int t = rt; t < T; t += rstep) {
    float pad = paddings ? bf16_bits_to_float(paddings[(long)b * T + t])
                         : 0.f;
    if (pad >= 0.5f) continue;
    const long base = ((long)b * T + t) * D + col0;
    ushortx8 xv = *reinterpret_cast<const ushortx8*>(x + base);
    ushortx8 dyv = *reinterpret_cast<const ushortx8*>(dy + base);
#pragma unroll
    for (int e = 0; e < 8; ++e) {
      float xf = bf16_bits_to_float(xv[e]);
      float df = bf16_bits_to_float(dyv[e]);
      float xhat = (xf - mu) * rs;
      if (act == 1) {
        const float ypre = xhat * w[e] + bb[e];
        const float sg = 1.f / (1.f + __expf(-ypre));
        df *= sg * (1.f + ypre * (1.f - sg));
      }
      float dxhat = df * w[e];
      s1 += dxhat;
      s2 += dxhat * xhat;
      dg8[e] += df * xhat;
      db8[e] += df;
    }
    count += 8.f;
  }
  __syncthreads();
  s1 = block_reduce_sum<GN_WAVES>(s1, scratch);
  s2 = block_reduce_sum<GN_WAVES>(s2, scratch);
  count = block_reduce_sum<GN_WAVES>(count, scratch);
  count = fmaxf(count, 1.f);
  const float inv_n = 1.f / count;
#pragma unroll
  for (int e = 0; e < 8; ++e) {
    if (dg8[e] != 0.f) atomicAdd(&dg_s[oct * 8 + e], dg8[e]);
    if (db8[e] != 0.f) atomicAdd(&db_s[oct * 8 + e], db8[e]);
  }
  __syncthreads();
  for (int i = tid; i < cg; i += GN_BLOCK) {
    int c = g * cg + i;
    if (dg_s[i] != 0.f) atomicAdd(dgamma + c, dg_s[i]);
    if (db_s[i] != 0.f) atomicAdd(dbeta + c, db_s[i]);
  }

  for (int t = rt; t < T; t += rstep) {
    float pad = paddings ? bf16_bits_to_float(paddings[(long)b * T + t])
                         : 0.f;
    const long base = ((long)b * T + t) * D + col0;
    ushortx8 xv = *reinterpret_cast<const ushortx8*>(x + base);
    ushortx8 dyv = *reinterpret_cast<const ushortx8*>(dy + base);
    ushortx8 o;
#pragma unroll
    for (int e = 0; e < 8; ++e) {
      float xf = bf16_bits_to_float(xv[e]);
      float df = bf16_bits_to_float(dyv[e]);
      float xhat = (xf - mu) * rs;
      if (act == 1) {
        const float ypre = xhat * w[e] + bb[e];
        const float sg = 1.f / (1.f + __expf(-ypre));
        df *= sg * (1.f + ypre * (1.f - sg));
      }
      float dxhat = df * w[e];
      float val = rs * (dxhat - inv_n * (s1 + xhat * s2)) * (1.f - pad);
      o[e] = float_to_bf16_bits(val);
    }
    *reinterpret_cast<ushortx8*>(dx + base) = o;
  }
}

}

std::vector<torch::Tensor> group_norm_fwd(torch::Tensor x,
                                          torch::Tensor gamma,
                                          torch::Tensor beta,
                                          c10::optional<torch::Tensor> pad,
                                          int64_t groups, double eps,
                                          int64_t act) {
  TORCH_CHECK(x.is_cuda() && x.is_contiguous() && x.dim() == 3 &&
              x.scalar_type() == torch::kBFloat16);
  const int B = x.size(0), T = x.size(1), D = x.size(2);
  const int G = (int)groups;
  TORCH_CHECK(D % G == 0 && D / G <= 64, "cg must be <= 64");
  auto y = torch::empty_like(x);
  auto opts = x.options().dtype(torch::kFloat32);
  auto mean = torch::empty({(long)B * G}, opts);
  auto rstd = torch::empty({(long)B * G}, opts);
  auto stream = at::cuda::getCurrentCUDAStream();
  TORCH_CHECK(act == 0 || (D / G) % 8 == 0,
              "fused activation needs cg % 8 == 0");
  hipLaunchKernelGGL(gn_fwd_kernel, dim3(B * G), dim3(GN_BLOCK), 0, stream,
                     (const unsigned short*)x.data_ptr(),
                     (const unsigned short*)gamma.data_ptr(),
                     (const unsigned short*)beta.data_ptr(),
                     pad.has_value()
                         ? (const unsigned short*)pad->data_ptr()
                         : nullptr,
                     (unsigned short*)y.data_ptr(), mean.data_ptr<float>(),
                     rstd.data_ptr<float>(), B, T, D, G, (float)eps,
                     (int)act);
  return {y, mean, rstd};
}

std::vector<torch::Tensor> group_norm_bwd(torch::Tensor dy, torch::Tensor x,
                                          torch::Tensor gamma,
                                          torch::Tensor beta,
                                          c10::optional<torch::Tensor> pad,
                                          torch::Tensor mean,
                                          torch::Tensor rstd,
                                          int64_t groups, int64_t act) {
  const int B = x.size(0), T = x.size(1), D = x.size(2);
  const int G = (int)groups;
  auto dx = torch::empty_like(x);
  auto opts = x.options().dtype(torch::kFloat32);
  auto dgamma = torch::zeros({D}, opts);
  auto dbeta = torch::zeros({D}, opts);
  auto stream = at::cuda::getCurrentCUDAStream();
  const int cg = D / G;
  const bool vec = cg % 8 == 0 && GN_BLOCK % (cg / 8) == 0;
  TORCH_CHECK(act == 0 || vec, "fused activation needs cg % 8 == 0");
  auto kern = vec ? gn_bwd_vec_kernel : gn_bwd_kernel;
  hipLaunchKernelGGL(kern, dim3(B * G), dim3(GN_BLOCK), 0, stream,
                     (const unsigned short*)dy.data_ptr(),
                     (const unsigned short*)x.data_ptr(),
                     (const unsigned short*)gamma.data_ptr(),
                     (const unsigned short*)beta.data_ptr(),
                     pad.has_value()
                         ? (const unsigned short*)pad->data_ptr()
                         : nullptr,
                     mean.data_ptr<float>(), rstd.data_ptr<float>(),
                     (unsigned short*)dx.data_ptr(),
                     dgamma.data_ptr<float>(), dbeta.data_ptr<float>(), B,
                     T, D, G, (int)act);
  return {dx, dgamma, dbeta};
}
```

Baseline: 1289 examples/sec.

## Fuse pointwise matmul, GLU, padding and depthwise conv; add tiled dwconv kernels

Replaces the pw1 matmul → GLU → padding → depthwise conv chain in the Conformer conv module with an autograd function. It runs the matmul through addmm, then one HIP kernel that applies GLU, the padding mask and the depthwise conv together, so the GLU output never goes to HBM. The backward pass also produces the pw1 bias gradient as column sums. The change also adds LDS-tiled depthwise conv kernels for the fwd, dx and dw passes, drops the old register variant, and adds a vectorized GroupNorm forward kernel. The aim is to cut memory traffic and kernel launches, at the cost of a lot of new kernel code and extra bindings.

```diff
diff --git a/lingvo_amd/core/py_utils.py b/lingvo_amd/core/py_utils.py
--- a/lingvo_amd/core/py_utils.py
+++ b/lingvo_amd/core/py_utils.py
@@ -478,6 +478,26 @@
                                  op_seed, scale=scale, paddings=paddings)
 
 
+def MatmulBiasGluDwconv(x: torch.Tensor, pw1_w: torch.Tensor,
+                        pw1_b: torch.Tensor,
+                        paddings: Optional[torch.Tensor],
+                        dw_w: torch.Tensor, dw_b: Optional[torch.Tensor],
+                        causal: bool = False) -> torch.Tensor:
+  d = dw_w.shape[-1]
+  if (GlueFusion() and x.is_cuda and x.dim() == 3 and x.numel() > 0 and
+      d % 8 == 0 and pw1_b is not None and pw1_w.shape[-1] == 2 * d and
+      all(t is None or t.dtype == torch.bfloat16
+          for t in (x, pw1_w, pw1_b, dw_w, dw_b))):
+    from lingvo_amd.ops import conv1d as conv1d_ops
+    return conv1d_ops.linear_glu_dwconv(x, pw1_w, pw1_b, paddings, dw_w,
+                                        dw_b, causal=causal)
+  from lingvo_amd.ops import conv1d as conv1d_ops
+  h = torch.nn.functional.glu(MatmulBias(x, pw1_w, pw1_b), dim=-1)
+  if paddings is not None:
+    h = ApplyPadding(paddings, h)
+  return conv1d_ops.depthwise_conv1d(h, dw_w, dw_b, causal=causal)
+
+
 class Timer:
 
   def __init__(self):
diff --git a/lingvo_amd/layers/conformer.py b/lingvo_amd/layers/conformer.py
--- a/lingvo_amd/layers/conformer.py
+++ b/lingvo_amd/layers/conformer.py
@@ -61,12 +61,9 @@
             paddings: Optional[torch.Tensor] = None) -> torch.Tensor:
     p = self.p
     x, residual = transformer_lib.PreLn(self.ln, theta.ln, inputs)
-    x = py_utils.MatmulBias(x, theta.pw1_w, theta.pw1_b)
-    x = F.glu(x, dim=-1)
-    if paddings is not None:
-      x = py_utils.ApplyPadding(paddings, x)
-    x = conv1d_ops.depthwise_conv1d(x, theta.dw_w, theta.dw_b,
-                                    causal=p.is_causal)
+    x = py_utils.MatmulBiasGluDwconv(x, theta.pw1_w, theta.pw1_b, paddings,
+                                     theta.dw_w, theta.dw_b,
+                                     causal=p.is_causal)
     if p.conv_norm == 'layer':
       x = self.norm.FProp(theta.norm, x)
       if paddings is not None:
diff --git a/lingvo_amd/ops/conv1d.py b/lingvo_amd/ops/conv1d.py
--- a/lingvo_amd/ops/conv1d.py
+++ b/lingvo_amd/ops/conv1d.py
@@ -8,15 +8,19 @@
 
 from lingvo_amd.ops import _loader
 
+def tile_len() -> int:
+  return int(_loader.get_ext(required=True).dwconv_tile_len())
+
 
 class _DwConv1dFn(torch.autograd.Function):
 
   @staticmethod
-  def forward(ctx, x, w, bias, pad):
+  def forward(ctx, x, w, bias, pad, route):
     ext = _loader.get_ext(required=True)
-    y = ext.dwconv1d_fwd(x, w, bias, pad)
+    y = ext.dwconv1d_fwd(x, w, bias, pad, route)
     ctx.save_for_backward(x, w)
     ctx.pad = pad
+    ctx.route = route
     ctx.has_bias = bias is not None
     ctx.wdtype = w.dtype
     return y
@@ -25,21 +29,27 @@
   def backward(ctx, dy):
     ext = _loader.get_ext(required=True)
     x, w = ctx.saved_tensors
-    dx, dw, db = ext.dwconv1d_bwd(dy.contiguous(), x, w, ctx.pad)
+    dx, dw, db = ext.dwconv1d_bwd(dy.contiguous(), x, w, ctx.pad, ctx.route)
     return (dx, dw.to(ctx.wdtype),
-            db.to(ctx.wdtype) if ctx.has_bias else None, None)
+            db.to(ctx.wdtype) if ctx.has_bias else None, None, None)
+
+
+def _pad_of(k: int, causal: bool) -> int:
+  return k - 1 if causal else (k - 1) // 2
 
 
 def depthwise_conv1d(x: torch.Tensor, w: torch.Tensor,
                      bias: Optional[torch.Tensor] = None,
-                     causal: bool = False) -> torch.Tensor:
+                     causal: bool = False,
+                     route: str = 'auto') -> torch.Tensor:
   k = w.shape[0]
-  pad = k - 1 if causal else (k - 1) // 2
+  pad = _pad_of(k, causal)
   if x.is_cuda:
     orig = x.dtype
     out = _DwConv1dFn.apply(
         x.to(torch.bfloat16).contiguous(), w.to(torch.bfloat16).contiguous(),
-        None if bias is None else bias.to(torch.bfloat16).contiguous(), pad)
+        None if bias is None else bias.to(torch.bfloat16).contiguous(), pad,
+        route)
     return out.to(orig) if orig != torch.bfloat16 else out
   xf = x.float().permute(0, 2, 1)
   wf = w.float().t().unsqueeze(1)
@@ -49,3 +59,84 @@
   out = F.conv1d(xf, wf, bias.float() if bias is not None else None,
                  groups=x.shape[2])
   return out.permute(0, 2, 1).to(x.dtype)
+
+
+def _bf16_pad(paddings: Optional[torch.Tensor],
+              like: torch.Tensor) -> Optional[torch.Tensor]:
+  if paddings is None:
+    return None
+  if paddings.dim() == 3 and paddings.shape[-1] == 1:
+    paddings = paddings.squeeze(-1)
+  if paddings.shape != like.shape[:2]:
+    raise ValueError(f'paddings must be [B,T]={tuple(like.shape[:2])}, got '
+                     f'{tuple(paddings.shape)}')
+  return paddings.to(torch.bfloat16).contiguous()
+
+
+class _GluDwConv1dFn(torch.autograd.Function):
+
+  @staticmethod
+  def forward(ctx, h, pad_mask, w, bias, pad):
+    ext = _loader.get_ext(required=True)
+    y = ext.glu_dwconv1d_fwd(h, pad_mask, w, bias, pad)
+    ctx.save_for_backward(h, w, *([] if pad_mask is None else [pad_mask]))
+    ctx.pad = pad
+    ctx.has_bias = bias is not None
+    return y
+
+  @staticmethod
+  def backward(ctx, dy):
+    ext = _loader.get_ext(required=True)
+    h, w, *rest = ctx.saved_tensors
+    dh, dw, db, _ = ext.glu_dwconv1d_bwd(dy.contiguous(), h,
+                                         rest[0] if rest else None, w, ctx.pad)
+    return (dh, None, dw.to(w.dtype),
+            db.to(w.dtype) if ctx.has_bias else None, None)
+
+
+def glu_depthwise_conv1d(h: torch.Tensor, paddings: Optional[torch.Tensor],
+                         w: torch.Tensor,
+                         bias: Optional[torch.Tensor] = None,
+                         causal: bool = False) -> torch.Tensor:
+  return _GluDwConv1dFn.apply(h, _bf16_pad(paddings, h), w, bias,
+                              _pad_of(w.shape[0], causal))
+
+
+class _LinearGluDwConvFn(torch.autograd.Function):
+
+  @staticmethod
+  def forward(ctx, x2, pw1_w, pw1_b, pad_mask, dw_w, dw_b, pad, bt):
+    ext = _loader.get_ext(required=True)
+    h = torch.addmm(pw1_b, x2, pw1_w).view(bt[0], bt[1], -1)
+    y = ext.glu_dwconv1d_fwd(h, pad_mask, dw_w, dw_b, pad)
+    ctx.save_for_backward(x2, pw1_w, h, dw_w,
+                          *([] if pad_mask is None else [pad_mask]))
+    ctx.pad = pad
+    ctx.has_bias = dw_b is not None
+    return y
+
+  @staticmethod
+  def backward(ctx, dy):
+    ext = _loader.get_ext(required=True)
+    x2, pw1_w, h, dw_w, *rest = ctx.saved_tensors
+    dh, ddw, ddb, dcol = ext.glu_dwconv1d_bwd(
+        dy.contiguous(), h, rest[0] if rest else None, dw_w, ctx.pad)
+    dh2 = dh.view(-1, dh.shape[-1])
+    dx = torch.mm(dh2, pw1_w.t()) if ctx.needs_input_grad[0] else None
+    dw1 = torch.mm(x2.t(), dh2) if ctx.needs_input_grad[1] else None
+    db1 = dcol.to(torch.bfloat16) if ctx.needs_input_grad[2] else None
+    return (dx, dw1, db1, None, ddw.to(dw_w.dtype),
+            ddb.to(dw_w.dtype) if ctx.has_bias else None, None, None)
+
+
+def linear_glu_dwconv(x: torch.Tensor, pw1_w: torch.Tensor,
+                      pw1_b: torch.Tensor, paddings: Optional[torch.Tensor],
+                      dw_w: torch.Tensor, dw_b: Optional[torch.Tensor],
+                      causal: bool = False) -> torch.Tensor:
+  assert x.is_cuda and x.dtype == torch.bfloat16 and x.dim() == 3
+  x2 = x.reshape(-1, x.shape[-1])
+  y = _LinearGluDwConvFn.apply(
+      x2, pw1_w, pw1_b, _bf16_pad(paddings, x), dw_w.contiguous(),
+      None if dw_b is None else dw_b.contiguous(),
+      _pad_of(dw_w.shape[0], causal), (x.shape[0], x.shape[1]))
+  return y
diff --git a/lingvo_amd/ops/hip/bindings.cpp b/lingvo_amd/ops/hip/bindings.cpp
--- a/lingvo_amd/ops/hip/bindings.cpp
+++ b/lingvo_amd/ops/hip/bindings.cpp
@@ -41,9 +41,27 @@
                                   const std::string& route);
 
 torch::Tensor dwconv1d_fwd(torch::Tensor x, torch::Tensor w,
-                           c10::optional<torch::Tensor> bias, int64_t pad);
-std::vector<torch::Tensor> dwconv1d_bwd(torch::Tensor dy, torch::Tensor x,
-                                        torch::Tensor w, int64_t pad);
+                           c10::optional<torch::Tensor> bias, int64_t pad,
+                           const std::string& route,
+                           c10::optional<torch::Tensor> y_out);
+std::vector<torch::Tensor> dwconv1d_bwd(
+    torch::Tensor dy, torch::Tensor x, torch::Tensor w, int64_t pad,
+    const std::string& route, c10::optional<torch::Tensor> dx_out,
+    c10::optional<torch::Tensor> dw_out, c10::optional<torch::Tensor> db_out);
+torch::Tensor glu_dwconv1d_fwd(torch::Tensor h,
+                               c10::optional<torch::Tensor> paddings,
+                               torch::Tensor w,
+                               c10::optional<torch::Tensor> bias, int64_t pad,
+                               const std::string& route,
+                               c10::optional<torch::Tensor> y_out);
+std::vector<torch::Tensor> glu_dwconv1d_bwd(
+    torch::Tensor dy, torch::Tensor h, c10::optional<torch::Tensor> paddings,
+    torch::Tensor w, int64_t pad, const std::string& route,
+    c10::optional<torch::Tensor> dh_out, c10::optional<torch::Tensor> dw_out,
+    c10::optional<torch::Tensor> db_out,
+    c10::optional<torch::Tensor> dcol_out);
+
+int64_t dwconv_tile_len();
 
 std::vector<torch::Tensor> xent_fwd(torch::Tensor logits,
                                     torch::Tensor labels);
@@ -70,7 +88,8 @@
                                           torch::Tensor beta,
                                           c10::optional<torch::Tensor> pad,
                                           int64_t groups, double eps,
-                                          int64_t act);
+                                          int64_t act,
+                                          const std::string& route);
 std::vector<torch::Tensor> group_norm_bwd(torch::Tensor dy, torch::Tensor x,
                                           torch::Tensor gamma,
                                           torch::Tensor beta,
@@ -163,7 +182,10 @@
   RegisterInputPipeline(m);
   RegisterWpmTokenizer(m);
   RegisterRecordBatcher(m);
-  m.def("group_norm_fwd", &group_norm_fwd, "Fused padded GroupNorm fwd");
+  m.def("group_norm_fwd", &group_norm_fwd, "Fused padded GroupNorm fwd",
+        py::arg("x"), py::arg("gamma"), py::arg("beta"), py::arg("pad"),
+        py::arg("groups"), py::arg("eps"), py::arg("act"),
+        py::arg("route") = "auto");
   m.def("group_norm_bwd", &group_norm_bwd, "Fused padded GroupNorm bwd");
   m.def("lstm_gates_fwd", &lstm_gates_fwd_op, "Fused LSTM gates fwd");
   m.def("lstm_gates_bwd", &lstm_gates_bwd_op, "Fused LSTM gates bwd");
@@ -173,8 +195,25 @@
         "Fused dropout bwd + fp32 column sums of dx");
   m.def("xent_fwd", &xent_fwd, "Fused softmax-xent fwd");
   m.def("xent_bwd", &xent_bwd, "Fused softmax-xent bwd");
-  m.def("dwconv1d_fwd", &dwconv1d_fwd, "Depthwise time conv fwd");
-  m.def("dwconv1d_bwd", &dwconv1d_bwd, "Depthwise time conv bwd");
+  m.def("dwconv1d_fwd", &dwconv1d_fwd, "Depthwise time conv fwd",
+        py::arg("x"), py::arg("w"), py::arg("bias"), py::arg("pad"),
+        py::arg("route") = "auto", py::arg("y_out") = py::none());
+  m.def("dwconv1d_bwd", &dwconv1d_bwd, "Depthwise time conv bwd",
+        py::arg("dy"), py::arg("x"), py::arg("w"), py::arg("pad"),
+        py::arg("route") = "auto", py::arg("dx_out") = py::none(),
+        py::arg("dw_out") = py::none(), py::arg("db_out") = py::none());
+  m.def("glu_dwconv1d_fwd", &glu_dwconv1d_fwd,
+        "conv(mask * glu(h)) + bias in one kernel", py::arg("h"),
+        py::arg("paddings"), py::arg("w"), py::arg("bias"), py::arg("pad"),
+        py::arg("route") = "auto", py::arg("y_out") = py::none());
+  m.def("glu_dwconv1d_bwd", &glu_dwconv1d_bwd,
+        "dh, dw, db and the fp32 column sums of dh of glu_dwconv1d_fwd",
+        py::arg("dy"), py::arg("h"), py::arg("paddings"), py::arg("w"),
+        py::arg("pad"), py::arg("route") = "auto",
+        py::arg("dh_out") = py::none(), py::arg("dw_out") = py::none(),
+        py::arg("db_out") = py::none(), py::arg("dcol_out") = py::none());
+  m.def("dwconv_tile_len", &dwconv_tile_len,
+        "Time rows per tile of the tiled depthwise convolution");
   m.def("layer_norm_fwd", &layer_norm_fwd, "Fused LayerNorm/RMSNorm fwd");
   m.def("layer_norm_bwd", &layer_norm_bwd, "Fused LayerNorm/RMSNorm bwd",
         py::arg("dy"), py::arg("x"), py::arg("scale"), py::arg("mean"),
diff --git a/lingvo_amd/ops/hip/common.h b/lingvo_amd/ops/hip/common.h
--- a/lingvo_amd/ops/hip/common.h
+++ b/lingvo_amd/ops/hip/common.h
@@ -78,3 +78,6 @@
   long want = (total_work + block_size - 1) / block_size;
   return (int)(want < cap_blocks ? (want > 0 ? want : 1) : cap_blocks);
 }
+
+void colsum_reduce(const float* partials, float* out, int nslab, long D,
+                   hipStream_t stream);
diff --git a/lingvo_amd/ops/hip/conv1d.hip b/lingvo_amd/ops/hip/conv1d.hip
--- a/lingvo_amd/ops/hip/conv1d.hip
+++ b/lingvo_amd/ops/hip/conv1d.hip
@@ -2,7 +2,11 @@
 #include <ATen/cuda/CUDAContext.h>
 #include <torch/extension.h>
 
+#include <array>
+#include <string>
+
 #include "common.h"
+#include "dwconv_tiled.h"
 
 namespace {
 
@@ -64,81 +68,6 @@
   }
 }
 
-template <int KT, int R>
-__global__ __launch_bounds__(256) void dwconv_fwd_reg(
-    const unsigned short* __restrict__ x,
-    const unsigned short* __restrict__ w,
-    const unsigned short* __restrict__ bias,
-    unsigned short* __restrict__ y, int B, int T, int D, int pad) {
-  const int dvec = D / 8;
-  const int tblks = (T + R - 1) / R;
-  const long nwork = (long)B * tblks * dvec;
-  for (long i = (long)blockIdx.x * blockDim.x + threadIdx.x; i < nwork;
-       i += (long)gridDim.x * blockDim.x) {
-    const int dv = (int)(i % dvec);
-    const long bt = i / dvec;
-    const int t0 = (int)(bt % tblks) * R;
-    const long b = bt / tblks;
-    ushortx8 wv[KT];
-#pragma unroll
-    for (int j = 0; j < KT; ++j) {
-      wv[j] = *reinterpret_cast<const ushortx8*>(w + j * D + dv * 8);
-    }
-    float acc[R][8];
-#pragma unroll
-    for (int r = 0; r < R; ++r) {
-      if (bias) {
-        ushortx8 bv = *reinterpret_cast<const ushortx8*>(bias + dv * 8);
-#pragma unroll
-        for (int e = 0; e < 8; ++e) acc[r][e] = bf16_bits_to_float(bv[e]);
-      } else {
-#pragma unroll
-        for (int e = 0; e < 8; ++e) acc[r][e] = 0.f;
-      }
-    }
-    const long rowbase = b * T;
-    auto loadx = [&](int t) -> ushortx8 {
-      ushortx8 v;
-      if (t >= 0 && t < T) {
-        v = *reinterpret_cast<const ushortx8*>(
-            x + (rowbase + t) * D + dv * 8);
-      } else {
-#pragma unroll
-        for (int e = 0; e < 8; ++e) v[e] = 0;
-      }
-      return v;
-    };
-    ushortx8 W[R];
-#pragma unroll
-    for (int r = 0; r < R; ++r) W[r] = loadx(t0 + r - pad);
-#pragma unroll
-    for (int j = 0; j < KT; ++j) {
-#pragma unroll
-      for (int r = 0; r < R; ++r) {
-#pragma unroll
-        for (int e = 0; e < 8; ++e) {
-          acc[r][e] += bf16_bits_to_float(W[r][e]) *
-                       bf16_bits_to_float(wv[j][e]);
-        }
-      }
-      if (j + 1 < KT) {
-#pragma unroll
-        for (int r = 0; r + 1 < R; ++r) W[r] = W[r + 1];
-        W[R - 1] = loadx(t0 + (R - 1) + (j + 1) - pad);
-      }
-    }
-#pragma unroll
-    for (int r = 0; r < R; ++r) {
-      const int t = t0 + r;
-      if (t >= T) continue;
-      ushortx8 ov;
-#pragma unroll
-      for (int e = 0; e < 8; ++e) ov[e] = float_to_bf16_bits(acc[r][e]);
-      *reinterpret_cast<ushortx8*>(y + (rowbase + t) * D + dv * 8) = ov;
-    }
-  }
-}
-
 template <int KT>
 __global__ void dwconv_bwd_dx(const unsigned short* __restrict__ dy,
                               const unsigned short* __restrict__ w,
@@ -332,76 +261,227 @@
 
 }
 
-torch::Tensor dwconv1d_fwd(torch::Tensor x, torch::Tensor w,
-                           c10::optional<torch::Tensor> bias, int64_t pad) {
-  TORCH_CHECK(x.is_cuda() && x.is_contiguous() && x.dim() == 3 &&
-              x.scalar_type() == torch::kBFloat16, "x must be bf16 [B,T,D]");
-  TORCH_CHECK(x.size(2) % 8 == 0, "D must be divisible by 8");
-  const int B = x.size(0), T = x.size(1), D = x.size(2), K = w.size(0);
-  TORCH_CHECK(K < MAXK, "kernel size < ", MAXK);
-  auto y = torch::empty_like(x);
-  auto stream = at::cuda::getCurrentCUDAStream();
-  long nvec = (long)B * T * (D / 8);
-  int grid = memory_bound_grid(nvec, 256);
-  static const bool use_reg = []() {
-    const char* e = getenv("LINGVO_DWCONV_REG");
-    return e && e[0] == '1';
-  }();
-  if (use_reg && K == 32) {
-    long nwork = (long)B * ((T + 3) / 4) * (D / 8);
-    hipLaunchKernelGGL((dwconv_fwd_reg<32, 4>),
-                       dim3(memory_bound_grid(nwork, 256)), dim3(256), 0,
-                       stream, (const unsigned short*)x.data_ptr(),
-                       (const unsigned short*)w.data_ptr(),
-                       bias.has_value() ? (const unsigned short*)
-                                              bias->data_ptr()
-                                        : nullptr,
-                       (unsigned short*)y.data_ptr(), B, T, D, (int)pad);
-    return y;
-  }
-  auto fwd_kern = dwconv_fwd<0>;
-  hipLaunchKernelGGL(fwd_kern, dim3(grid), dim3(256), 0, stream,
-                     (const unsigned short*)x.data_ptr(),
-                     (const unsigned short*)w.data_ptr(),
-                     bias.has_value() ? (const unsigned short*)
-                                            bias->data_ptr()
-                                      : nullptr,
-                     (unsigned short*)y.data_ptr(), B, T, D, K, (int)pad);
-  return y;
-}
-
-std::vector<torch::Tensor> dwconv1d_bwd(torch::Tensor dy, torch::Tensor x,
-                                        torch::Tensor w, int64_t pad) {
-  const int B = x.size(0), T = x.size(1), D = x.size(2), K = w.size(0);
-  auto dx = torch::empty_like(x);
-  auto opts = x.options().dtype(torch::kFloat32);
-  auto dw = torch::zeros({K, D}, opts);
-  auto db = torch::zeros({D}, opts);
-  auto stream = at::cuda::getCurrentCUDAStream();
-  long nvec = (long)B * T * (D / 8);
-  auto dx_kern = dwconv_bwd_dx<0>;
-  hipLaunchKernelGGL(dx_kern, dim3(memory_bound_grid(nvec, 256)),
-                     dim3(256), 0, stream,
-                     (const unsigned short*)dy.data_ptr(),
-                     (const unsigned short*)w.data_ptr(),
-                     (unsigned short*)dx.data_ptr(), B, T, D, K, (int)pad);
+namespace {
+
+const unsigned short* bf16_ptr(const torch::Tensor& t) {
+  return (const unsigned short*)t.data_ptr();
+}
+
+const unsigned short* opt_ptr(const c10::optional<torch::Tensor>& t) {
+  return t.has_value() ? bf16_ptr(*t) : nullptr;
+}
+
+bool is_bf16_cuda(const torch::Tensor& t) {
+  return t.is_cuda() && t.is_contiguous() &&
+         t.scalar_type() == torch::kBFloat16;
+}
+
+bool pick_tiled(const std::string& route, int64_t B, int64_t T, int64_t D,
+                int64_t K) {
+  if (route == "naive") return false;
+  const bool ok = dwconv_tiled_supported(B, T, D, K);
+  if (route == "auto") return ok;
+  TORCH_CHECK(route == "tiled",
+              "route must be 'auto', 'naive' or 'tiled', got '", route, "'");
+  TORCH_CHECK(ok, "route='tiled' does not support B=", B, " T=", T, " D=", D,
+              " K=", K);
+  return true;
+}
+
+torch::Tensor out_or_empty(const c10::optional<torch::Tensor>& out,
+                           at::IntArrayRef sizes,
+                           const torch::TensorOptions& opts,
+                           const char* name) {
+  if (!out.has_value()) return torch::empty(sizes, opts);
+  TORCH_CHECK(out->is_cuda() && out->is_contiguous() &&
+              out->scalar_type() == opts.dtype().toScalarType() &&
+              out->sizes() == sizes &&
+              reinterpret_cast<uintptr_t>(out->data_ptr()) % 16 == 0,
+              name, " must be a contiguous 16-byte aligned tensor of shape ",
+              sizes);
+  return *out;
+}
+
+void check_conv_args(const torch::Tensor& x, const torch::Tensor& w,
+                     const c10::optional<torch::Tensor>& bias, int64_t D,
+                     int64_t pad) {
+  TORCH_CHECK(D % 8 == 0, "D must be divisible by 8");
+  TORCH_CHECK(is_bf16_cuda(w) && w.dim() == 2 && w.size(1) == D,
+              "w must be contiguous bf16 [K,D]");
+  const int64_t K = w.size(0);
+  TORCH_CHECK(K >= 1 && K < MAXK, "kernel size < ", MAXK);
+  TORCH_CHECK(pad >= 0 && pad < K, "pad must be in [0, K)");
+  TORCH_CHECK(!bias.has_value() ||
+              (is_bf16_cuda(*bias) && bias->dim() == 1 && bias->size(0) == D),
+              "bias must be contiguous bf16 [D]");
+}
+
+void launch_bwd_dw(bool tiled, bool glu, const torch::Tensor& dy,
+                   const torch::Tensor& x, const unsigned short* padm,
+                   torch::Tensor& dw, torch::Tensor& db, int B, int T, int D,
+                   int K, int pad, hipStream_t stream) {
+  TORCH_CHECK(tiled || !glu, "the naive weight gradient takes u, not h");
+  auto opts = dw.options();
   long nchunks = ((long)B * T + DW_CHUNK - 1) / DW_CHUNK;
   int dblks = (D + DW_DBLK - 1) / DW_DBLK;
-  int ngroups = (int)std::min<long>(std::max<long>(1, 1024 / dblks),
-                                    nchunks);
+  int ngroups = tiled ? (int)dwconv_tiled_dw_groups(B, T, D)
+                      : (int)std::min<long>(
+                            std::max<long>(1, 1024 / dblks), nchunks);
   auto dw_part = torch::empty({(long)ngroups * K * D}, opts);
   auto db_part = torch::empty({(long)ngroups * D}, opts);
-  dim3 grid_w(dblks, ngroups);
-  hipLaunchKernelGGL(dwconv_bwd_dw, grid_w, dim3(256), 0, stream,
-                     (const unsigned short*)dy.data_ptr(),
-                     (const unsigned short*)x.data_ptr(),
-                     dw_part.data_ptr<float>(), db_part.data_ptr<float>(),
-                     B, T, D, K, (int)pad, ngroups);
+  if (tiled) {
+    dwconv_tiled_dw(glu, bf16_ptr(dy), bf16_ptr(x), padm,
+                    dw_part.data_ptr<float>(), db_part.data_ptr<float>(), B,
+                    T, D, K, pad, ngroups, stream);
+  } else {
+    dim3 grid_w(dblks, ngroups);
+    hipLaunchKernelGGL(dwconv_bwd_dw, grid_w, dim3(256), 0, stream,
+                       bf16_ptr(dy), bf16_ptr(x), dw_part.data_ptr<float>(),
+                       db_part.data_ptr<float>(), B, T, D, K, pad, ngroups);
+  }
   const long kd = (long)K * D;
   hipLaunchKernelGGL(dwconv_bwd_dw_reduce,
                      dim3((int)std::min<long>((kd + D + 255) / 256, 1024)),
                      dim3(256), 0, stream, dw_part.data_ptr<float>(),
                      db_part.data_ptr<float>(), dw.data_ptr<float>(),
                      db.data_ptr<float>(), kd, D, ngroups);
+}
+
+}
+
+torch::Tensor dwconv1d_fwd(torch::Tensor x, torch::Tensor w,
+                           c10::optional<torch::Tensor> bias, int64_t pad,
+                           const std::string& route,
+                           c10::optional<torch::Tensor> y_out) {
+  TORCH_CHECK(is_bf16_cuda(x) && x.dim() == 3, "x must be bf16 [B,T,D]");
+  const int B = x.size(0), T = x.size(1), D = x.size(2);
+  check_conv_args(x, w, bias, D, pad);
+  const int K = w.size(0);
+  if (x.numel() == 0) return out_or_empty(y_out, x.sizes(), x.options(), "y_out");
+  const bool tiled = pick_tiled(route, B, T, D, K);
+  auto y = out_or_empty(y_out, x.sizes(), x.options(), "y_out");
+  auto stream = at::cuda::getCurrentCUDAStream();
+  if (tiled) {
+    dwconv_tiled_fwd(bf16_ptr(x), bf16_ptr(w), opt_ptr(bias),
+                     (unsigned short*)y.data_ptr(), B, T, D, K, (int)pad,
+                     stream);
+    return y;
+  }
+  long nvec = (long)B * T * (D / 8);
+  auto fwd_kern = dwconv_fwd<0>;
+  hipLaunchKernelGGL(fwd_kern, dim3(memory_bound_grid(nvec, 256)), dim3(256),
+                     0, stream, bf16_ptr(x), bf16_ptr(w), opt_ptr(bias),
+                     (unsigned short*)y.data_ptr(), B, T, D, K, (int)pad);
+  return y;
+}
+
+std::vector<torch::Tensor> dwconv1d_bwd(
+    torch::Tensor dy, torch::Tensor x, torch::Tensor w, int64_t pad,
+    const std::string& route, c10::optional<torch::Tensor> dx_out,
+    c10::optional<torch::Tensor> dw_out,
+    c10::optional<torch::Tensor> db_out) {
+  TORCH_CHECK(is_bf16_cuda(x) && x.dim() == 3, "x must be bf16 [B,T,D]");
+  TORCH_CHECK(is_bf16_cuda(dy) && dy.sizes() == x.sizes(),
+              "dy must be contiguous bf16 shaped like x");
+  const int B = x.size(0), T = x.size(1), D = x.size(2);
+  check_conv_args(x, w, c10::nullopt, D, pad);
+  const int K = w.size(0);
+  auto opts = x.options().dtype(torch::kFloat32);
+  if (x.numel() == 0) {
+    auto dx = out_or_empty(dx_out, x.sizes(), x.options(), "dx_out");
+    auto dw = out_or_empty(dw_out, {K, D}, opts, "dw_out");
+    auto db = out_or_empty(db_out, {D}, opts, "db_out");
+    return {dx, dw.zero_(), db.zero_()};
+  }
+  const bool tiled = pick_tiled(route, B, T, D, K);
+  auto dx = out_or_empty(dx_out, x.sizes(), x.options(), "dx_out");
+  auto dw = out_or_empty(dw_out, {K, D}, opts, "dw_out");
+  auto db = out_or_empty(db_out, {D}, opts, "db_out");
+  auto stream = at::cuda::getCurrentCUDAStream();
+  if (tiled) {
+    dwconv_tiled_dx(bf16_ptr(dy), bf16_ptr(w), (unsigned short*)dx.data_ptr(),
+                    B, T, D, K, (int)pad, stream);
+  } else {
+    long nvec = (long)B * T * (D / 8);
+    auto dx_kern = dwconv_bwd_dx<0>;
+    hipLaunchKernelGGL(dx_kern, dim3(memory_bound_grid(nvec, 256)), dim3(256),
+                       0, stream, bf16_ptr(dy), bf16_ptr(w),
+                       (unsigned short*)dx.data_ptr(), B, T, D, K, (int)pad);
+  }
+  launch_bwd_dw(tiled, false, dy, x, nullptr, dw, db, B, T, D, K, (int)pad,
+                stream);
   return {dx, dw, db};
 }
+
+namespace {
+
+std::array<int, 4> check_glu_args(const torch::Tensor& h,
+                                  const c10::optional<torch::Tensor>& paddings,
+                                  const torch::Tensor& w,
+                                  const c10::optional<torch::Tensor>& bias,
+                                  int64_t pad) {
+  TORCH_CHECK(h.is_cuda() && h.dim() == 3 &&
+              h.scalar_type() == torch::kBFloat16, "h must be bf16 [B,T,2D]");
+  TORCH_CHECK(h.is_contiguous(), "h must be contiguous");
+  TORCH_CHECK(w.dim() == 2 && h.size(2) == 2 * w.size(1),
+              "h.shape[-1] must be 2*D with w [K,D]");
+  const int64_t D = w.size(1);
+  check_conv_args(h, w, bias, D, pad);
+  TORCH_CHECK(h.numel() > 0, "empty input");
+  TORCH_CHECK(!paddings.has_value() ||
+              (is_bf16_cuda(*paddings) && paddings->dim() == 2 &&
+               paddings->size(0) == h.size(0) &&
+               paddings->size(1) == h.size(1)),
+              "paddings must be contiguous bf16 [B,T]");
+  return {(int)h.size(0), (int)h.size(1), (int)D, (int)w.size(0)};
+}
+
+}
+
+torch::Tensor glu_dwconv1d_fwd(torch::Tensor h,
+                               c10::optional<torch::Tensor> paddings,
+                               torch::Tensor w,
+                               c10::optional<torch::Tensor> bias, int64_t pad,
+                               const std::string& route,
+                               c10::optional<torch::Tensor> y_out) {
+  const auto s = check_glu_args(h, paddings, w, bias, pad);
+  const int B = s[0], T = s[1], D = s[2], K = s[3];
+  TORCH_CHECK(route != "naive", "the fused front has no naive route");
+  pick_tiled(route == "auto" ? "tiled" : route, B, T, D, K);
+  auto y = out_or_empty(y_out, {B, T, D}, h.options(), "y_out");
+  glu_dwconv_tiled_fwd(bf16_ptr(h), opt_ptr(paddings), bf16_ptr(w),
+                       opt_ptr(bias), (unsigned short*)y.data_ptr(), B, T, D,
+                       K, (int)pad, at::cuda::getCurrentCUDAStream());
+  return y;
+}
+
+std::vector<torch::Tensor> glu_dwconv1d_bwd(
+    torch::Tensor dy, torch::Tensor h, c10::optional<torch::Tensor> paddings,
+    torch::Tensor w, int64_t pad, const std::string& route,
+    c10::optional<torch::Tensor> dh_out, c10::optional<torch::Tensor> dw_out,
+    c10::optional<torch::Tensor> db_out,
+    c10::optional<torch::Tensor> dcol_out) {
+  const auto s = check_glu_args(h, paddings, w, c10::nullopt, pad);
+  const int B = s[0], T = s[1], D = s[2], K = s[3];
+  TORCH_CHECK(is_bf16_cuda(dy) && dy.dim() == 3 && dy.size(0) == B &&
+              dy.size(1) == T && dy.size(2) == D,
+              "dy must be contiguous bf16 [B,T,D]");
+  TORCH_CHECK(route != "naive", "the fused front has no naive route");
+  pick_tiled(route == "auto" ? "tiled" : route, B, T, D, K);
+  auto opts = h.options().dtype(torch::kFloat32);
+  auto dh = out_or_empty(dh_out, {B, T, 2 * D}, h.options(), "dh_out");
+  auto dw = out_or_empty(dw_out, {K, D}, opts, "dw_out");
+  auto db = out_or_empty(db_out, {D}, opts, "db_out");
+  auto dcol = out_or_empty(dcol_out, {2 * D}, opts, "dcol_out");
+  const int groups = (int)dwconv_tiled_groups(B, T);
+  auto cs_part = torch::empty({groups, 2 * D}, opts);
+  auto stream = at::cuda::getCurrentCUDAStream();
+  glu_dwconv_tiled_dx(bf16_ptr(dy), bf16_ptr(h), opt_ptr(paddings),
+                      bf16_ptr(w), (unsigned short*)dh.data_ptr(),
+                      cs_part.data_ptr<float>(), B, T, D, K, (int)pad, stream);
+  colsum_reduce(cs_part.data_ptr<float>(), dcol.data_ptr<float>(), groups,
+                2L * D, stream);
+  launch_bwd_dw(true, true, dy, h, opt_ptr(paddings), dw, db, B, T, D, K,
+                (int)pad, stream);
+  return {dh, dw, db, dcol};
+}
diff --git a/lingvo_amd/ops/hip/dropout.hip b/lingvo_amd/ops/hip/dropout.hip
--- a/lingvo_amd/ops/hip/dropout.hip
+++ b/lingvo_amd/ops/hip/dropout.hip
@@ -187,6 +187,12 @@
   }
 }
 
+}
+
+void colsum_reduce(const float* partials, float* out, int nslab, long D,
+                   hipStream_t stream) {
+  hipLaunchKernelGGL(colsum_reduce_kernel, dim3(cdiv(D, 16)), dim3(256), 0,
+                     stream, partials, out, nslab, D);
 }
 
 torch::Tensor dropout_fwd(torch::Tensor x, c10::optional<torch::Tensor> res,
@@ -318,8 +324,7 @@
     LAUNCH_BWD_CS(0);
   }
 #undef LAUNCH_BWD_CS
-  hipLaunchKernelGGL(colsum_reduce_kernel, dim3(cdiv(d, 16)), dim3(256), 0,
-                     stream, partials.data_ptr<float>(),
-                     colsum.data_ptr<float>(), gy, (long)d);
+  colsum_reduce(partials.data_ptr<float>(), colsum.data_ptr<float>(), gy,
+                (long)d, stream);
   return {dx, colsum};
 }
diff --git a/lingvo_amd/ops/hip/dwconv_tiled.h b/lingvo_amd/ops/hip/dwconv_tiled.h
--- /dev/null
+++ b/lingvo_amd/ops/hip/dwconv_tiled.h
@@ -0,0 +1,30 @@
+#pragma once
+
+#include <hip/hip_runtime.h>
+
+#include <cstdint>
+
+int64_t dwconv_tile_len();
+int64_t dwconv_tiled_groups(int64_t B, int64_t T);
+bool dwconv_tiled_supported(int64_t B, int64_t T, int64_t D, int64_t K);
+
+int64_t dwconv_tiled_dw_groups(int64_t B, int64_t T, int64_t D);
+void dwconv_tiled_dw(bool glu, const unsigned short* dy,
+                     const unsigned short* x, const unsigned short* padm,
+                     float* dw_part, float* db_part, int B, int T, int D,
+                     int K, int pad, int ngroups, hipStream_t stream);
+void dwconv_tiled_fwd(const unsigned short* x, const unsigned short* w,
+                      const unsigned short* bias, unsigned short* y, int B,
+                      int T, int D, int K, int pad,
+                      hipStream_t stream);
+void dwconv_tiled_dx(const unsigned short* dy, const unsigned short* w,
+                     unsigned short* dx, int B, int T, int D, int K, int pad,
+                     hipStream_t stream);
+void glu_dwconv_tiled_fwd(const unsigned short* h, const unsigned short* padm,
+                          const unsigned short* w, const unsigned short* bias,
+                          unsigned short* y, int B, int T, int D, int K,
+                          int pad, hipStream_t stream);
+void glu_dwconv_tiled_dx(const unsigned short* dy, const unsigned short* h,
+                         const unsigned short* padm, const unsigned short* w,
+                         unsigned short* dh, float* cs_part, int B, int T,
+                         int D, int K, int pad, hipStream_t stream);
diff --git a/lingvo_amd/ops/hip/dwconv_tiled.hip b/lingvo_amd/ops/hip/dwconv_tiled.hip
--- /dev/null
+++ b/lingvo_amd/ops/hip/dwconv_tiled.hip
@@ -0,0 +1,419 @@
+
+#include <ATen/cuda/CUDAContext.h>
+#include <torch/extension.h>
+
+#include <algorithm>
+
+#include "common.h"
+#include "dwconv_tiled.h"
+
+namespace {
+
+typedef __attribute__((ext_vector_type(2))) float floatx2;
+
+enum { kPlainFwd = 0, kPlainDx = 1, kGluFwd = 2, kGluDx = 3 };
+
+template <int KT_, int R_, int CB_, int NT_>
+struct TileCfg {
+  static constexpr int KT = KT_;
+  static constexpr int R = R_;
+  static constexpr int CB = CB_;
+  static constexpr int NT = NT_;
+  static constexpr int NP = CB / 2;
+  static constexpr int NRG = NT / NP;
+  static constexpr int TT = R * NRG;
+  static constexpr int OCT = CB / 8;
+  static constexpr int NRL = NT / OCT;
+  static constexpr int IN_ROWS = TT + KT - 1;
+  static constexpr int IN_BYTES = IN_ROWS * CB * 2;
+  static constexpr int OUT_BYTES = TT * CB * 4;
+  static constexpr int RED_BYTES = NRL * 2 * CB * 4;
+  static constexpr int LDS_BYTES =
+      IN_BYTES > OUT_BYTES ? (IN_BYTES > RED_BYTES ? IN_BYTES : RED_BYTES)
+                           : (OUT_BYTES > RED_BYTES ? OUT_BYTES : RED_BYTES);
+  static constexpr int DW_LDS_BYTES =
+      IN_BYTES + TT * CB * 2 + (KT + 1) * CB * 4;
+  static_assert(NT % NP == 0 && NT % OCT == 0 && CB % 8 == 0, "tile shape");
+  static_assert(LDS_BYTES <= 64 * 1024 && DW_LDS_BYTES <= 64 * 1024,
+                "static LDS limit");
+};
+
+__device__ __forceinline__ float sigmoidf_(float g) {
+  return 1.f / (1.f + expf(-g));
+}
+
+__device__ __forceinline__ float keep_of(unsigned short p) {
+  return bf16_bits_to_float(float_to_bf16_bits(1.f - bf16_bits_to_float(p)));
+}
+
+template <bool GLU, int ROWS, class C>
+__device__ __forceinline__ void stage_rows(
+    const unsigned short* __restrict__ in, long in_stride,
+    const unsigned short* __restrict__ padm, unsigned short* in_s, long b,
+    int T, int D, int t_first, int d0, int tid) {
+  constexpr int CB = C::CB, NT = C::NT;
+  constexpr int kStage = (ROWS * C::OCT + NT - 1) / NT;
+#pragma unroll
+  for (int it = 0; it < kStage; ++it) {
+    const int idx = tid + it * NT;
+    const int row = idx / C::OCT;
+    const int o = idx % C::OCT;
+    const int t = t_first + row;
+    const int gd = d0 + o * 8;
+    const bool ok = t >= 0 && t < T && gd < D;
+    const long grow = b * T + (ok ? t : 0);
+    const int gdc = ok ? gd : 0;
+    ushortx8 v = *reinterpret_cast<const ushortx8*>(in + grow * in_stride + gdc);
+    if (GLU) {
+      const ushortx8 gv = *reinterpret_cast<const ushortx8*>(
+          in + grow * in_stride + D + gdc);
+      const float keep = padm ? keep_of(padm[grow]) : 1.f;
+#pragma unroll
+      for (int e = 0; e < 8; ++e) {
+        const unsigned short u = float_to_bf16_bits(
+            bf16_bits_to_float(v[e]) * sigmoidf_(bf16_bits_to_float(gv[e])));
+        v[e] = padm ? float_to_bf16_bits(bf16_bits_to_float(u) * keep) : u;
+      }
+    }
+    if (!ok) {
+#pragma unroll
+      for (int e = 0; e < 8; ++e) v[e] = 0;
+    }
+    if (idx < ROWS * C::OCT)
+      *reinterpret_cast<ushortx8*>(in_s + row * CB + o * 8) = v;
+  }
+}
+
+template <int MODE, class C>
+__global__ __launch_bounds__(C::NT) void dwconv_tiled_kernel(
+    const unsigned short* __restrict__ in,
+    const unsigned short* __restrict__ h,
+    const unsigned short* __restrict__ padm,
+    const unsigned short* __restrict__ w,
+    const unsigned short* __restrict__ bias,
+    unsigned short* __restrict__ out,
+    float* __restrict__ cs_part,
+    int T, int D, int K, int pad, int ntt, int ndb) {
+  constexpr int KT = C::KT, R = C::R, CB = C::CB, NT = C::NT;
+  constexpr bool kFlip = MODE == kPlainDx || MODE == kGluDx;
+  __shared__ __attribute__((aligned(16))) unsigned char lds[C::LDS_BYTES];
+  unsigned short* in_s = reinterpret_cast<unsigned short*>(lds);
+  float* out_s = reinterpret_cast<float*>(lds);
+
+  const int tid = threadIdx.x;
+  const int db = blockIdx.x % ndb;
+  const int tile = blockIdx.x / ndb;
+  const int tt = tile % ntt;
+  const long b = tile / ntt;
+  const int t0 = tt * C::TT;
+  const int d0 = db * CB;
+  const int epad = kFlip ? K - 1 - pad : pad;
+  const long in_stride = MODE == kGluFwd ? 2L * D : D;
+
+  const int p = tid % C::NP;
+  const int rg = tid / C::NP;
+  const int dp = d0 + 2 * p;
+  floatx2 wt[KT];
+#pragma unroll
+  for (int j = 0; j < KT; ++j) {
+    const int jj = kFlip ? K - 1 - j : j;
+    const bool ok = j < K && dp < D;
+    const unsigned int v = *reinterpret_cast<const unsigned int*>(
+        w + (ok ? (long)jj * D + dp : 0L));
+    wt[j][0] = ok ? __uint_as_float(v << 16) : 0.f;
+    wt[j][1] = ok ? __uint_as_float(v & 0xffff0000u) : 0.f;
+  }
+
+  stage_rows<MODE == kGluFwd, C::IN_ROWS, C>(in, in_stride, padm, in_s, b, T,
+                                             D, t0 - epad, d0, tid);
+  __syncthreads();
+
+  floatx2 acc[R];
+  {
+    floatx2 b2 = {0.f, 0.f};
+    if (!kFlip && bias && dp < D) {
+      const unsigned int v = *reinterpret_cast<const unsigned int*>(bias + dp);
+      b2[0] = __uint_as_float(v << 16);
+      b2[1] = __uint_as_float(v & 0xffff0000u);
+    }
+#pragma unroll
+    for (int r = 0; r < R; ++r) acc[r] = b2;
+  }
+  const unsigned short* base = in_s + (rg * R) * CB + 2 * p;
+#pragma unroll
+  for (int i = 0; i < R + KT - 1; ++i) {
+    const unsigned int v = *reinterpret_cast<const unsigned int*>(base + i * CB);
+    floatx2 xv;
+    xv[0] = __uint_as_float(v << 16);
+    xv[1] = __uint_as_float(v & 0xffff0000u);
+#pragma unroll
+    for (int r = 0; r < R; ++r) {
+      const int j = i - r;
+      if (j >= 0 && j < KT) acc[r] += xv * wt[j];
+    }
+  }
+  __syncthreads();
+#pragma unroll
+  for (int r = 0; r < R; ++r)
+    *reinterpret_cast<floatx2*>(out_s + (rg * R + r) * CB + 2 * p) = acc[r];
+  __syncthreads();
+
+  const int o = tid % C::OCT;
+  const int rl = tid / C::OCT;
+  const int gd = d0 + o * 8;
+  float csa[8], csg[8];
+#pragma unroll
+  for (int e = 0; e < 8; ++e) csa[e] = csg[e] = 0.f;
+  for (int row = rl; row < C::TT; row += C::NRL) {
+    const int t = t0 + row;
+    if (t >= T || gd >= D) break;
+    const floatx4 lo = *reinterpret_cast<const floatx4*>(out_s + row * CB + o * 8);
+    const floatx4 hi =
+        *reinterpret_cast<const floatx4*>(out_s + row * CB + o * 8 + 4);
+    const float r8[8] = {lo[0], lo[1], lo[2], lo[3], hi[0], hi[1], hi[2], hi[3]};
+    const long grow = b * T + t;
+    if (MODE != kGluDx) {
+      ushortx8 ov;
+#pragma unroll
+      for (int e = 0; e < 8; ++e) ov[e] = float_to_bf16_bits(r8[e]);
+      *reinterpret_cast<ushortx8*>(out + grow * D + gd) = ov;
+    } else {
+      const ushortx8 av =
+          *reinterpret_cast<const ushortx8*>(h + grow * 2L * D + gd);
+      const ushortx8 gv =
+          *reinterpret_cast<const ushortx8*>(h + grow * 2L * D + D + gd);
+      const float keep = padm ? keep_of(padm[grow]) : 1.f;
+      ushortx8 oa, og;
+#pragma unroll
+      for (int e = 0; e < 8; ++e) {
+        const float s = sigmoidf_(bf16_bits_to_float(gv[e]));
+        const float du = keep == 0.f ? 0.f : r8[e] * keep;
+        oa[e] = float_to_bf16_bits(du * s);
+        og[e] = float_to_bf16_bits(du * bf16_bits_to_float(av[e]) * s *
+                                   (1.f - s));
+        csa[e] += bf16_bits_to_float(oa[e]);
+        csg[e] += bf16_bits_to_float(og[e]);
+      }
+      *reinterpret_cast<ushortx8*>(out + grow * 2L * D + gd) = oa;
+      *reinterpret_cast<ushortx8*>(out + grow * 2L * D + D + gd) = og;
+    }
+  }
+  if (MODE == kGluDx) {
+    __syncthreads();
+    float* red = reinterpret_cast<float*>(lds);
+#pragma unroll
+    for (int e = 0; e < 8; ++e) {
+      red[(rl * 2 + 0) * CB + o * 8 + e] = csa[e];
+      red[(rl * 2 + 1) * CB + o * 8 + e] = csg[e];
+    }
+    __syncthreads();
+    for (int c = tid; c < 2 * CB; c += NT) {
+      const int half = c / CB, cc = c % CB;
+      if (d0 + cc < D) {
+        float s = 0.f;
+        for (int q = 0; q < C::NRL; ++q) s += red[(q * 2 + half) * CB + cc];
+        cs_part[(long)tile * 2 * D + (long)half * D + d0 + cc] = s;
+      }
+    }
+  }
+}
+
+template <bool GLU, class C>
+__global__ __launch_bounds__(C::NT) void dwconv_tiled_dw_kernel(
+    const unsigned short* __restrict__ dy,
+    const unsigned short* __restrict__ x,
+    const unsigned short* __restrict__ padm,
+    float* __restrict__ dw_part, float* __restrict__ db_part, int T, int D,
+    int K, int pad, int ntt, int ndb, int ntiles, int ngroups) {
+  constexpr int KT = C::KT, R = C::R, CB = C::CB, NT = C::NT;
+  __shared__ __attribute__((aligned(16))) unsigned short in_s[C::IN_ROWS * CB];
+  __shared__ __attribute__((aligned(16))) unsigned short dy_s[C::TT * CB];
+  __shared__ float red[(KT + 1) * CB];
+  const int tid = threadIdx.x;
+  const int db = blockIdx.x % ndb;
+  const int grp = blockIdx.x / ndb;
+  const int d0 = db * CB;
+  const int p = tid % C::NP;
+  const int rg = tid / C::NP;
+  const long in_stride = GLU ? 2L * D : D;
+
+  floatx2 acc[KT];
+#pragma unroll
+  for (int j = 0; j < KT; ++j) acc[j] = floatx2{0.f, 0.f};
+  floatx2 dbacc = {0.f, 0.f};
+
+  for (int tile = grp; tile < ntiles; tile += ngroups) {
+    const int tt = tile % ntt;
+    const long b = tile / ntt;
+    const int t0 = tt * C::TT;
+    stage_rows<GLU, C::IN_ROWS, C>(x, in_stride, padm, in_s, b, T, D,
+                                   t0 - pad, d0, tid);
+    stage_rows<false, C::TT, C>(dy, D, nullptr, dy_s, b, T, D, t0, d0, tid);
+    __syncthreads();
+    floatx2 g[R];
+#pragma unroll
+    for (int r = 0; r < R; ++r) {
+      const unsigned int v = *reinterpret_cast<const unsigned int*>(
+          dy_s + (rg * R + r) * CB + 2 * p);
+      g[r][0] = __uint_as_float(v << 16);
+      g[r][1] = __uint_as_float(v & 0xffff0000u);
+      dbacc += g[r];
+    }
+    const unsigned short* base = in_s + (rg * R) * CB + 2 * p;
+#pragma unroll
+    for (int i = 0; i < R + KT - 1; ++i) {
+      const unsigned int v =
+          *reinterpret_cast<const unsigned int*>(base + i * CB);
+      floatx2 xv;
+      xv[0] = __uint_as_float(v << 16);
+      xv[1] = __uint_as_float(v & 0xffff0000u);
+#pragma unroll
+      for (int r = 0; r < R; ++r) {
+        const int j = i - r;
+        if (j >= 0 && j < KT) acc[j] += g[r] * xv;
+      }
+    }
+    __syncthreads();
+  }
+
+  for (int q = 0; q < C::NRG; ++q) {
+    if (rg == q) {
+#pragma unroll
+      for (int j = 0; j < KT; ++j) {
+        floatx2* dst = reinterpret_cast<floatx2*>(red + j * CB + 2 * p);
+        *dst = q == 0 ? acc[j] : *dst + acc[j];
+      }
+      floatx2* dst = reinterpret_cast<floatx2*>(red + KT * CB + 2 * p);
+      *dst = q == 0 ? dbacc : *dst + dbacc;
+    }
+    __syncthreads();
+  }
+  for (int i = tid; i < K * CB; i += NT) {
+    const int j = i / CB, c = i % CB;
+    if (d0 + c < D)
+      dw_part[((long)grp * K + j) * D + d0 + c] = red[j * CB + c];
+  }
+  for (int c = tid; c < CB; c += NT) {
+    if (d0 + c < D) db_part[(long)grp * D + d0 + c] = red[KT * CB + c];
+  }
+}
+
+using Cfg0 = TileCfg<32, 20, 64, 256>;
+using Cfg0K16 = TileCfg<16, 20, 64, 256>;
+using Cfg0K8 = TileCfg<8, 20, 64, 256>;
+
+int lds_limit() {
+  static const int limit = []() {
+    int dev = 0, v = 0;
+    LV_CHECK_HIP(hipGetDevice(&dev));
+    LV_CHECK_HIP(hipDeviceGetAttribute(
+        &v, hipDeviceAttributeMaxSharedMemoryPerBlock, dev));
+    return v;
+  }();
+  return limit;
+}
+
+template <int MODE, class C>
+void launch(const unsigned short* in, const unsigned short* h,
+            const unsigned short* padm, const unsigned short* w,
+            const unsigned short* bias, unsigned short* out, float* cs_part,
+            int B, int T, int D, int K, int pad, hipStream_t stream) {
+  const int ntt = (T + C::TT - 1) / C::TT;
+  const int ndb = (D + C::CB - 1) / C::CB;
+  hipLaunchKernelGGL((dwconv_tiled_kernel<MODE, C>),
+                     dim3((unsigned)((long)B * ntt * ndb)), dim3(C::NT), 0,
+                     stream, in, h, padm, w, bias, out, cs_part, T, D, K, pad,
+                     ntt, ndb);
+}
+
+template <int MODE>
+void dispatch(const unsigned short* in, const unsigned short* h,
+              const unsigned short* padm, const unsigned short* w,
+              const unsigned short* bias, unsigned short* out, float* cs_part,
+              int B, int T, int D, int K, int pad, hipStream_t stream) {
+#define LV_GO(C) \
+  launch<MODE, C>(in, h, padm, w, bias, out, cs_part, B, T, D, K, pad, stream)
+  if (K <= 8) {
+    LV_GO(Cfg0K8);
+  } else if (K <= 16) {
+    LV_GO(Cfg0K16);
+  } else {
+    LV_GO(Cfg0);
+  }
+#undef LV_GO
+}
+
+}
+
+int64_t dwconv_tile_len() { return Cfg0::TT; }
+
+int64_t dwconv_tiled_groups(int64_t B, int64_t T) {
+  const int tt = Cfg0::TT;
+  return B * ((T + tt - 1) / tt);
+}
+
+bool dwconv_tiled_supported(int64_t B, int64_t T, int64_t D, int64_t K) {
+  if (B < 1 || T < 1 || D < 8 || D % 8 != 0 || K < 1 || K > 32) return false;
+  const long tiles = B * ((T + Cfg0::TT - 1) / Cfg0::TT) *
+                     ((D + Cfg0::CB - 1) / Cfg0::CB);
+  if (tiles >= (1L << 31)) return false;
+  return Cfg0::LDS_BYTES <= lds_limit() && Cfg0::DW_LDS_BYTES <= lds_limit();
+}
+
+int64_t dwconv_tiled_dw_groups(int64_t B, int64_t T, int64_t D) {
+  const long ntiles = B * ((T + Cfg0::TT - 1) / Cfg0::TT);
+  const long ndb = (D + Cfg0::CB - 1) / Cfg0::CB;
+  return std::min<long>(ntiles, std::max<long>(1, 1536 / ndb));
+}
+
+void dwconv_tiled_dw(bool glu, const unsigned short* dy,
+                     const unsigned short* x, const unsigned short* padm,
+                     float* dw_part, float* db_part, int B, int T, int D,
+                     int K, int pad, int ngroups, hipStream_t stream) {
+  const int ntt = (T + Cfg0::TT - 1) / Cfg0::TT;
+  const int ndb = (D + Cfg0::CB - 1) / Cfg0::CB;
+#define LV_DW(GLU, C)                                                        \
+  hipLaunchKernelGGL((dwconv_tiled_dw_kernel<GLU, C>),                       \
+                     dim3((unsigned)((long)ngroups * ndb)), dim3(C::NT), 0,  \
+                     stream, dy, x, padm, dw_part, db_part, T, D, K, pad,    \
+                     ntt, ndb, B * ntt, ngroups)
+  if (K <= 8) {
+    if (glu) LV_DW(true, Cfg0K8); else LV_DW(false, Cfg0K8);
+  } else if (K <= 16) {
+    if (glu) LV_DW(true, Cfg0K16); else LV_DW(false, Cfg0K16);
+  } else {
+    if (glu) LV_DW(true, Cfg0); else LV_DW(false, Cfg0);
+  }
+#undef LV_DW
+}
+
+void dwconv_tiled_fwd(const unsigned short* x, const unsigned short* w,
+                      const unsigned short* bias, unsigned short* y, int B,
+                      int T, int D, int K, int pad,
+                      hipStream_t stream) {
+  dispatch<kPlainFwd>(x, nullptr, nullptr, w, bias, y, nullptr, B, T, D,
+                      K, pad, stream);
+}
+
+void dwconv_tiled_dx(const unsigned short* dy, const unsigned short* w,
+                     unsigned short* dx, int B, int T, int D, int K, int pad,
+                     hipStream_t stream) {
+  dispatch<kPlainDx>(dy, nullptr, nullptr, w, nullptr, dx, nullptr, B, T,
+                     D, K, pad, stream);
+}
+
+void glu_dwconv_tiled_fwd(const unsigned short* h, const unsigned short* padm,
+                          const unsigned short* w, const unsigned short* bias,
+                          unsigned short* y, int B, int T, int D, int K,
+                          int pad, hipStream_t stream) {
+  dispatch<kGluFwd>(h, nullptr, padm, w, bias, y, nullptr, B, T, D, K,
+                    pad, stream);
+}
+
+void glu_dwconv_tiled_dx(const unsigned short* dy, const unsigned short* h,
+                         const unsigned short* padm, const unsigned short* w,
+                         unsigned short* dh, float* cs_part, int B, int T,
+                         int D, int K, int pad, hipStream_t stream) {
+  dispatch<kGluDx>(dy, h, padm, w, nullptr, dh, cs_part, B, T, D, K, pad,
+                   stream);
+}
diff --git a/lingvo_amd/ops/hip/group_norm.hip b/lingvo_amd/ops/hip/group_norm.hip
--- a/lingvo_amd/ops/hip/group_norm.hip
+++ b/lingvo_amd/ops/hip/group_norm.hip
@@ -1,6 +1,8 @@
 
 #include <ATen/cuda/CUDAContext.h>
 #include <torch/extension.h>
+
+#include <string>
 
 #include "common.h"
 
@@ -60,6 +62,80 @@
     if (act == 1) out = out / (1.f + __expf(-out));
     out *= (1.f - pad);
     y[((long)b * T + t) * D + c] = float_to_bf16_bits(out);
+  }
+}
+
+__global__ __launch_bounds__(GN_BLOCK) void gn_fwd_vec_kernel(
+    const unsigned short* __restrict__ x,
+    const unsigned short* __restrict__ gamma,
+    const unsigned short* __restrict__ beta,
+    const unsigned short* __restrict__ paddings,
+    unsigned short* __restrict__ y, float* __restrict__ mean_out,
+    float* __restrict__ rstd_out, int B, int T, int D, int G, float eps,
+    int act) {
+  __shared__ float scratch[GN_WAVES];
+  const int b = blockIdx.x / G;
+  const int g = blockIdx.x % G;
+  const int cg = D / G;
+  const int noct = cg / 8;
+  const int tid = threadIdx.x;
+  const int oct = tid % noct;
+  const int rt = tid / noct;
+  const int rstep = GN_BLOCK / noct;
+  const int t_first = rt < rstep ? rt : T;
+  const long col0 = (long)g * cg + (rt < rstep ? oct : 0) * 8;
+
+  float sum = 0.f, sumsq = 0.f, count = 0.f;
+  for (int t = t_first; t < T; t += rstep) {
+    const float pad =
+        paddings ? bf16_bits_to_float(paddings[(long)b * T + t]) : 0.f;
+    if (pad >= 0.5f) continue;
+    const ushortx8 xv = *reinterpret_cast<const ushortx8*>(
+        x + ((long)b * T + t) * D + col0);
+#pragma unroll
+    for (int e = 0; e < 8; ++e) {
+      const float v = bf16_bits_to_float(xv[e]);
+      sum += v;
+      sumsq += v * v;
+    }
+    count += 8.f;
+  }
+  sum = block_reduce_sum<GN_WAVES>(sum, scratch);
+  sumsq = block_reduce_sum<GN_WAVES>(sumsq, scratch);
+  count = block_reduce_sum<GN_WAVES>(count, scratch);
+  count = fmaxf(count, 1.f);
+  const float mu = sum / count;
+  const float var = sumsq / count - mu * mu;
+  const float rstd = rsqrtf(var + eps);
+  if (tid == 0) {
+    mean_out[(long)b * G + g] = mu;
+    rstd_out[(long)b * G + g] = rstd;
+  }
+
+  float w[8], bb[8];
+  {
+    const ushortx8 gv = *reinterpret_cast<const ushortx8*>(gamma + col0);
+    const ushortx8 bv = *reinterpret_cast<const ushortx8*>(beta + col0);
+#pragma unroll
+    for (int e = 0; e < 8; ++e) {
+      w[e] = 1.f + bf16_bits_to_float(gv[e]);
+      bb[e] = bf16_bits_to_float(bv[e]);
+    }
+  }
+  for (int t = t_first; t < T; t += rstep) {
+    const float pad =
+        paddings ? bf16_bits_to_float(paddings[(long)b * T + t]) : 0.f;
+    const long base = ((long)b * T + t) * D + col0;
+    const ushortx8 xv = *reinterpret_cast<const ushortx8*>(x + base);
+    ushortx8 o;
+#pragma unroll
+    for (int e = 0; e < 8; ++e) {
+      float out = (bf16_bits_to_float(xv[e]) - mu) * rstd * w[e] + bb[e];
+      if (act == 1) out = out / (1.f + __expf(-out));
+      out *= (1.f - pad);
+      o[e] = float_to_bf16_bits(out);
+    }
+    *reinterpret_cast<ushortx8*>(y + base) = o;
   }
 }
 
@@ -255,12 +331,18 @@
                                           torch::Tensor beta,
                                           c10::optional<torch::Tensor> pad,
                                           int64_t groups, double eps,
-                                          int64_t act) {
+                                          int64_t act,
+                                          const std::string& route) {
   TORCH_CHECK(x.is_cuda() && x.is_contiguous() && x.dim() == 3 &&
               x.scalar_type() == torch::kBFloat16);
   const int B = x.size(0), T = x.size(1), D = x.size(2);
   const int G = (int)groups;
   TORCH_CHECK(D % G == 0 && D / G <= 64, "cg must be <= 64");
+  TORCH_CHECK(route == "auto" || route == "scalar" || route == "vec",
+              "route must be 'auto', 'scalar' or 'vec'");
+  const bool can_vec = (D / G) % 8 == 0;
+  TORCH_CHECK(route != "vec" || can_vec, "route='vec' needs cg % 8 == 0");
+  const bool vec = can_vec && route != "scalar";
   auto y = torch::empty_like(x);
   auto opts = x.options().dtype(torch::kFloat32);
   auto mean = torch::empty({(long)B * G}, opts);
@@ -268,7 +350,8 @@
   auto stream = at::cuda::getCurrentCUDAStream();
   TORCH_CHECK(act == 0 || (D / G) % 8 == 0,
               "fused activation needs cg % 8 == 0");
-  hipLaunchKernelGGL(gn_fwd_kernel, dim3(B * G), dim3(GN_BLOCK), 0, stream,
+  hipLaunchKernelGGL(vec ? gn_fwd_vec_kernel : gn_fwd_kernel, dim3(B * G),
+                     dim3(GN_BLOCK), 0, stream,
                      (const unsigned short*)x.data_ptr(),
                      (const unsigned short*)gamma.data_ptr(),
                      (const unsigned short*)beta.data_ptr(),
```

Measured after the change: 1385 examples/sec (median of 6 runs). 1.07x the previous value.
